# maoqingyu1996/Boosting-Neural-Video-Representation-via-Online-Structural-Reparameteration

Measured on AMD Instinct MI355X. Metric: training frames/sec, Bunny 720p ERB, higher is better.
Workload: dtype f16; 1 GPU; configs[1]: Bunny-shaped 132x3x720x1280 synthetic video, branch_type=ERB, fc_hw_dim 9_16_26, strides 5 2 2 2 2, stem 512_1, lower_width 96, Fusion6, Adam(0.5,0.999), b=1; one independent video per GPU; precision=fp16, hip_graph=False, launch_mode=stream, finite=True

## Files before the change

boosting-neural-video-representation-via-online-structural-reparameteration_amd/csrc/orn_engine.hip:

```cpp
#include "orn_internal.h"
#include <new>
#include <cstdlib>
#include <cassert>

struct LayerBuf {
    float *T, *wf, *bf;
    float *w2t;
    float *dT, *dw1p;
    float *wd32;
    void *mh16;
    float *dw2t;
    float *z, *a;
    float *da;
    uint16_t *xpad;
    uint16_t *zb;
    uint16_t *dypad;
    uint16_t *wb, *wd;
    float *biasp;
    float *wslab;
};

struct orn_engine {
    orn_engine_desc d;
    float *params, *grads, *m, *v;
    const float *gmask;
    const float *tstats;
    float *ws;
    float *pre1, *h1, *pre2, *h2, *dh2;
    float *img, *dimg, *stats;
    float *loss_ws;
    float *dec_ws;
    float *scratch;
    float *head_ws;
    OrnStepCur *cur;
    LayerBuf L[ORN_MAX_LAYERS];
    int Hout, Wout, Cn_last;
    const OrnHalfOps *ops;
    float gs;
    OrnScaleState *sc;
    struct MergeSet {
        int n;
        OrnMergeLayer ml[ORN_MAX_LAYERS];
        int layer[ORN_MAX_LAYERS];
        void *tables;
        int tiles[4];
        void *mh_tables, *mh_host;
    } mset[3];
    int ff;
    float *dxn;
    size_t stem_ws;
    bool stage0;
    hipGraph_t graph, graph_u;
    hipGraphExec_t graph_exec, graph_exec_u;
    const void *g_frames, *g_embeds, *g_sched, *g_cursor, *g_stats;
    int g_slots;
    hipStream_t g_stream;
    hipStream_t side;
    hipEvent_t ev_fork, ev_adam, ev_wgrad, ev_join, ev_below;
    OrnStepCur *cur_side;
    OrnScaleState *sc_side;
    size_t side_lo;
    bool pipe_ok;
    bool side_below;
    bool fork_behind_dgrad;
    int last_smax;
    bool side_busy;
    bool prof;
    hipEvent_t prof_ev[4 * ORN_MAX_LAYERS + 4];
};

#define ORN_GRAPH_UNROLL 4
static_assert(ORN_SCALE_SLOTS >= ORN_GRAPH_UNROLL, "one scale-state entry per step of the unrolled graph");

static inline size_t al(size_t floats) { return orn_align(floats * 4) / 4; }

static hipEvent_t orn_engine::*const SIDE_EVENTS[] = {&orn_engine::ev_fork, &orn_engine::ev_adam, &orn_engine::ev_wgrad, &orn_engine::ev_join,
                                                      &orn_engine::ev_below};

static constexpr int ORN_LAST_SMAX = 24;

static void drop_graphs(orn_engine *e)
{
    if (e->graph_exec) { (void)hipGraphExecDestroy(e->graph_exec); e->graph_exec = nullptr; }
    if (e->graph) { (void)hipGraphDestroy(e->graph); e->graph = nullptr; }
    if (e->graph_exec_u) { (void)hipGraphExecDestroy(e->graph_exec_u); e->graph_exec_u = nullptr; }
    if (e->graph_u) { (void)hipGraphDestroy(e->graph_u); e->graph_u = nullptr; }
}

extern "C" size_t orn_conv3x3_ps_silu_bwd_ws_bytes(int B, int C, int O, int H, int W);
extern "C" size_t orn_erb_merge_bwd_ws_bytes(int C, int O);
extern "C" size_t orn_head_bwd_ws_bytes(int B, int C, int H, int W);
extern "C" size_t orn_loss_ws_bytes(int B, int Ch, int H, int W);

static int check_desc(const orn_engine_desc *d)
{
    ORN_REQUIRE(d, "engine: null desc");
    ORN_REQUIRE(d->n_layers >= 1 && d->n_layers <= ORN_MAX_LAYERS, "engine: n_layers=%d out of range", d->n_layers);
    ORN_REQUIRE(d->precision >= 0 && d->precision <= 2, "engine: precision %d not built", d->precision);
    ORN_REQUIRE(d->embed_len > 0 && d->stem_dim > 0 && d->fc_h > 0 && d->fc_w > 0 && d->fc_dim > 0, "engine: bad stem geometry");
    int C = d->fc_dim, H = d->fc_h, W = d->fc_w;
    for (int i = 0; i < d->n_layers; ++i) {
        const orn_layer_desc &l = d->layer[i];
        ORN_REQUIRE(l.C == C && l.H == H && l.W == W,
                    "engine: layer %d geometry (C=%d,H=%d,W=%d) does not chain (expected %d,%d,%d)", i, l.C, l.H, l.W, C, H, W);
        ORN_REQUIRE(l.s >= 1 && l.O > 0 && l.O % (l.s * l.s) == 0, "engine: layer %d: O=%d not divisible by s^2", i, l.O);
        ORN_REQUIRE(l.w3x3 >= 0 && l.b3x3 >= 0, "engine: layer %d: missing 3x3 weight/bias", i);
        if (d->erb)
            ORN_REQUIRE(l.w3x1 >= 0 && l.b3x1 >= 0 && l.w1x3 >= 0 && l.b1x3 >= 0 && l.w1 >= 0 && l.w2 >= 0 && l.w3 >= 0,
                        "engine: layer %d: missing ERB branch tensors", i);
        C = l.O / (l.s * l.s); H *= l.s; W *= l.s;
    }
    ORN_REQUIRE(d->n_params > 0 && d->n_params % 4 == 0, "engine: n_params must be a positive multiple of 4");
    ORN_REQUIRE(d->loss_type >= 0 && d->loss_type <= 2, "engine: bad loss_type %d", d->loss_type);
    return 0;
}

#define ORN_FAST_C 96
static bool layer_is_fast(const orn_layer_desc &l)
{
    return l.C == ORN_FAST_C && l.O % 96 == 0 && l.O % (l.s * l.s) == 0;
}

static int first_fast_layer(const orn_engine_desc *d)
{
    if (d->precision == 0) return d->n_layers;
    const orn_layer_desc &last = d->layer[d->n_layers - 1];
    const int cn = last.O / (last.s * last.s);
    if (!(cn == 32 || cn == 64 || cn == 96 || cn == 128)) return d->n_layers;
    int ff = d->n_layers;
    while (ff > 0 && layer_is_fast(d->layer[ff - 1])) --ff;
    if (ff > 0 && ff < d->n_layers) {
        const orn_layer_desc &l = d->layer[ff - 1];
        if (l.C < ORN_FAST_C && l.O % 96 == 0 && l.O % (l.s * l.s) == 0) --ff;
    }
    return ff;
}

static size_t layout(const orn_engine_desc *d, orn_engine *e)
{
    size_t off = 0;
    const int ff = first_fast_layer(d);
    float *dxn = nullptr;
    float *base = e ? e->ws : nullptr;
    auto take = [&](size_t floats) { float *p = base ? base + off : nullptr; off += al(floats); return p; };
    const int Nout = d->fc_h * d->fc_w * d->fc_dim;
    float *pre1 = take(d->stem_dim), *h1 = take(d->stem_dim), *pre2 = take(Nout), *h2 = take(Nout), *dh2 = take(Nout);
    size_t scratch = orn_stem_bwd_ws_floats(1, d->stem_dim, Nout);
    LayerBuf L[ORN_MAX_LAYERS] = {};
    int Cn = d->fc_dim, H = d->fc_h, W = d->fc_w;
    for (int i = 0; i < d->n_layers; ++i) {
        const orn_layer_desc &l = d->layer[i];
        const size_t wsz = (size_t)l.O * l.C * 9;
        if (d->erb) {
            L[i].T = take(wsz); L[i].wf = take(wsz); L[i].bf = take(l.O);
            L[i].w2t = (2 * l.C * 9 * 4 * 4 <= 64 * 1024) ? take((size_t)9 * l.O * 2 * l.C) : nullptr;
            L[i].dT = take(wsz); L[i].dw1p = take((size_t)9 * 2 * l.C * l.C);
            if (d->precision != 0) {
                L[i].mh16 = take((orn_merge_h16_layer_halfs(l.C, l.O) + 1) / 2);
                L[i].dw2t = take((size_t)9 * l.O * 2 * l.C);
            }
        }
        Cn = l.O / (l.s * l.s); H = l.H * l.s; W = l.W * l.s;
        const size_t asz = (size_t)Cn * H * W;
        size_t s1;
        if (i < ff) {
            L[i].z = take(asz); L[i].a = take(asz); L[i].da = take(asz);
            L[i].wd32 = take(wsz);
            s1 = orn_conv3x3_ps_silu_bwd_ws_bytes(1, l.C, l.O, l.H, l.W) / 4;
            const size_t s0 = al(orn_stem_bwd_ws_floats(1, d->stem_dim, Nout)) + (size_t)orn_stage0_slabs(l.O, l.s) * l.C * l.H * l.W;
            if (s0 > s1) s1 = s0;
        } else {
            const size_t wpz = (size_t)l.O * ORN_FAST_C * 9 + 96 * ORN_FAST_C;
            L[i].xpad = (uint16_t *)take(((size_t)(l.H + 2) * (l.W + 2) * ORN_FAST_C + 1) / 2);
            L[i].zb = (uint16_t *)take((asz + 1) / 2);
            L[i].dypad = (uint16_t *)take(((size_t)(l.H + 2) * (l.W + 2) * l.O + 128 + 1) / 2);
            L[i].wb = (uint16_t *)take((wpz + 1) / 2);
            L[i].wd = (uint16_t *)take((wpz + 1) / 2);
            L[i].biasp = take(l.O);
            L[i].wslab = take(orn_half_ops_bf16()->wgrad_ws_floats(l.H, l.W, l.O));
            const OrnHalfOps *ops = orn_half_ops_bf16();
            if (i == ff) dxn = take((size_t)l.H * l.W * ORN_FAST_C * ops->dgrad_f32_slabs(l.H, l.W, l.O));
            s1 = al(ops->wgrad_ws_floats(l.H, l.W, l.O));
            const size_t sd = (size_t)l.H * l.W * ORN_FAST_C * ops->dgrad_f32_slabs(l.H, l.W, l.O);
            if (ops->dgrad_f32_slabs(l.H, l.W, l.O) > 1 && sd > s1) s1 = sd;
        }
        if (d->erb) { const size_t s2 = orn_erb_merge_bwd_ws_bytes(l.C, l.O) / 4; if (s2 > s1) s1 = s2; }
        if (s1 > scratch) scratch = s1;
    }
    const size_t isz = (size_t)3 * H * W;
    float *img = take(isz), *dimg = take(isz), *stats = take(8);
    float *loss_ws = take(orn_loss_ws_bytes(1, 3, H, W) / 4);
    const size_t s3 = (ff < d->n_layers) ? orn_half_ops_bf16()->head_bwd_ws_floats(Cn) : orn_head_bwd_ws_bytes(1, Cn, H, W) / 4;
    if (s3 > scratch) scratch = s3;
    float *scr = take(scratch);
    const orn_layer_desc &ll = d->layer[d->n_layers - 1];
    float *head_ws = (ff < d->n_layers) ? take(orn_half_ops_bf16()->head_bwd_ws_floats(Cn))
                   : (ll.s == 2 ? take((size_t)(orn_head_bwd_fused_f32_blocks(ll.H, ll.W) + 1) * (3 * Cn + 3)) : nullptr);
    float *cur = take((sizeof(OrnStepCur) * ORN_GRAPH_UNROLL + 3) / 4 + 16);
    float *scs = take(sizeof(OrnScaleState) * ORN_SCALE_SLOTS / 4);
    float *mtab[3], *mhtab[3];
    for (int k = 0; k < 3; ++k) {
        mtab[k] = d->erb ? take(orn_merge_group_bytes() / 4) : nullptr;
        mhtab[k] = (d->erb && d->precision != 0) ? take(orn_merge_h16_table_bytes() / 4) : nullptr;
    }
    float *cur_side = take((sizeof(OrnStepCur) + 3) / 4 + 16);
    float *sc_side = take(sizeof(OrnScaleState) / 4 + 16);
    float *dec_ws = take(ORN_DECODE_WS_FLOATS);
    if (e) {
        e->pre1 = pre1; e->h1 = h1; e->pre2 = pre2; e->h2 = h2; e->dh2 = dh2;
        e->img = img; e->dimg = dimg; e->stats = stats; e->loss_ws = loss_ws; e->scratch = scr; e->head_ws = head_ws;
        e->cur = (OrnStepCur *)cur;
        e->sc = (OrnScaleState *)scs;
        for (int i = 0; i < d->n_layers; ++i) e->L[i] = L[i];
        e->Hout = H; e->Wout = W; e->Cn_last = Cn;
        e->ff = ff; e->dxn = dxn;
        e->stem_ws = al(orn_stem_bwd_ws_floats(1, d->stem_dim, Nout));
        const orn_layer_desc &l0 = d->layer[0];
        e->stage0 = d->precision != 0 && ff == 1 && d->n_layers > 1 && orn_stage0_supported(l0.C, l0.O, l0.H, l0.W, l0.s);
        for (int k = 0; k < 3; ++k) { e->mset[k].tables = mtab[k]; e->mset[k].mh_tables = mhtab[k]; }
        e->cur_side = (OrnStepCur *)cur_side;
        e->sc_side = (OrnScaleState *)sc_side;
        e->dec_ws = dec_ws;
    }
    return off * 4;
}

extern "C" size_t orn_engine_ws_bytes(const orn_engine_desc *d)
{
    if (check_desc(d) != 0) return 0;
    return layout(d, nullptr);
}

extern "C" int orn_engine_create(const orn_engine_desc *d, float *params, float *grads, float *adam_m, float *adam_v,
                                 void *ws, size_t ws_bytes, orn_engine **out)
{
    ORN_TRY(check_desc(d));
    ORN_REQUIRE(params && out && ws, "engine_create: null pointer");
    ORN_REQUIRE(((uintptr_t)params | (uintptr_t)grads | (uintptr_t)adam_m | (uintptr_t)adam_v | (uintptr_t)ws) % 256 == 0,
                "engine_create: arenas and workspace must be 256-byte aligned");
    const size_t need = layout(d, nullptr);
    if (ws_bytes < need) {
        orn_set_error("engine_create: workspace %zu < %zu", ws_bytes, need);
        return ORN_E_WS;
    }
    ORN_TRY(orn_loss_init());
    orn_engine *e = new (std::nothrow) orn_engine();
    ORN_REQUIRE(e, "engine_create: out of host memory");
    e->d = *d;
    e->params = params; e->grads = grads; e->m = adam_m; e->v = adam_v;
    e->gmask = nullptr;
    e->tstats = nullptr;
    e->ws = (float *)ws;
    e->graph = nullptr; e->graph_exec = nullptr; e->graph_u = nullptr; e->graph_exec_u = nullptr;
    e->prof = false;
    for (int k = 0; k < 3; ++k) { e->mset[k].n = 0; e->mset[k].mh_host = nullptr; }
    e->side = nullptr;
    for (auto ev : SIDE_EVENTS) e->*ev = nullptr;
    e->pipe_ok = false; e->side_busy = false; e->side_lo = 0;
    for (int i = 0; i < 4 * ORN_MAX_LAYERS + 4; ++i) e->prof_ev[i] = nullptr;
    e->ops = (d->precision == 2) ? orn_half_ops_f16() : orn_half_ops_bf16();
    e->gs = (d->precision == 2) ? 1048576.0f : 1.0f;
    layout(d, e);
    {
        hipError_t rc = hipMemset(ws, 0, need);
        if (rc == hipSuccess) rc = hipDeviceSynchronize();
        if (rc != hipSuccess) { orn_set_error("engine_create: hipMemset failed: %s", hipGetErrorString(rc)); delete e; return (int)rc; }
        OrnScaleState s0[ORN_SCALE_SLOTS] = {};
        for (int r = 0; r < ORN_SCALE_SLOTS; ++r) { s0[r].gs = e->gs; s0[r].inv_gs = 1.0f / e->gs; s0[r].gs_max = e->gs; }
        rc = hipMemcpy(e->sc, s0, sizeof(s0), hipMemcpyHostToDevice);
        if (rc == hipSuccess) rc = hipMemcpy(e->sc_side, s0, sizeof(OrnScaleState), hipMemcpyHostToDevice);
        if (rc != hipSuccess) { orn_set_error("engine_create: scale state upload failed: %s", hipGetErrorString(rc)); delete e; return (int)rc; }
    }
    {
        const int nl = d->n_layers;
        const orn_layer_desc &ll = d->layer[nl - 1];
        bool ok = d->precision != 0 && e->ff < nl - 1 && grads && adam_m && adam_v;
        if (ok) {
            const int64_t lo_all[9] = {ll.w3x3, ll.b3x3, ll.w3x1, ll.b3x1, ll.w1x3, ll.b1x3, ll.w1, ll.w2, ll.w3};
            int64_t lo = d->n_params;
            for (int k = 0; k < (d->erb ? 9 : 2); ++k) if (lo_all[k] >= 0 && lo_all[k] < lo) lo = lo_all[k];
            ok = d->head_w >= lo && d->head_b >= lo && d->stem_w0 < lo && d->stem_b0 < lo && d->stem_w1 < lo && d->stem_b1 < lo && lo % 64 == 0;
            for (int i = 0; i < nl - 1 && ok; ++i) {
                const orn_layer_desc &l = d->layer[i];
                const int64_t o[9] = {l.w3x3, l.b3x3, l.w3x1, l.b3x1, l.w1x3, l.b1x3, l.w1, l.w2, l.w3};
                for (int k = 0; k < (d->erb ? 9 : 2); ++k) ok = ok && o[k] < lo;
            }
            e->side_lo = (size_t)lo;
        }
        if (ok) {
            hipError_t rc = hipStreamCreateWithFlags(&e->side, hipStreamNonBlocking);
            for (auto ev : SIDE_EVENTS)
                if (rc == hipSuccess) rc = hipEventCreateWithFlags(&(e->*ev), hipEventDisableTiming | hipEventDisableSystemFence);
            if (rc != hipSuccess) { orn_set_error("engine_create: side stream: %s", hipGetErrorString(rc)); orn_engine_destroy(e); return (int)rc; }
        }
        e->pipe_ok = ok;
        e->last_smax = ok ? ORN_LAST_SMAX : 0;
        e->side_below = ok && nl - 2 > e->ff;
        e->fork_behind_dgrad = e->side_below;
    }
    if (!d->erb)
        for (int i = 0; i < d->n_layers; ++i) {
            e->L[i].T = nullptr;
            e->L[i].wf = params + d->layer[i].w3x3;
            e->L[i].bf = params + d->layer[i].b3x3;
        }
    else {
        auto fill = [&](int i, OrnMergeLayer &m, bool half_in_S) {
            const orn_layer_desc &l = d->layer[i];
            m.C = l.C; m.O = l.O;
            m.w3x3 = params + l.w3x3; m.w3x1 = params + l.w3x1; m.w1x3 = params + l.w1x3;
            m.w1 = params + l.w1; m.w2 = params + l.w2; m.w3 = params + l.w3;
            m.T = e->L[i].T; m.wf = e->L[i].wf; m.w2t = e->L[i].w2t;
            m.b3x3 = params + l.b3x3; m.b1x3 = params + l.b1x3; m.b3x1 = params + l.b3x1; m.bf = e->L[i].bf;
            m.g = grads ? grads + l.w3x3 : nullptr;
            m.dT = e->L[i].dT; m.dw1p = e->L[i].dw1p;
            m.dw2 = grads ? grads + l.w2 : nullptr; m.dw3 = grads ? grads + l.w3 : nullptr;
            m.dw2t = e->L[i].dw2t;
            m.half_kind = 0; m.s2 = l.s * l.s; m.Cp = ORN_FAST_C; m.wb = m.wd = nullptr; m.biasp = nullptr;
            if (i >= e->ff && half_in_S) {
                m.half_kind = d->precision; m.wb = e->L[i].wb; m.wd = e->L[i].wd; m.biasp = e->L[i].biasp;
            }
        };
        const int nl = d->n_layers;
        for (int k = 0; k < (e->pipe_ok ? 3 : 1); ++k) {
            orn_engine::MergeSet &ms = e->mset[k];
            const int i0 = k == 2 ? nl - 1 : 0, i1 = k == 1 ? nl - 1 : nl;
            ms.n = 0;
            void *bufs[ORN_MAX_LAYERS];
            for (int i = i0; i < i1; ++i) {
                fill(i, ms.ml[ms.n], k == 2 || !e->stage0);
                bufs[ms.n] = e->L[i].mh16;
                ms.layer[ms.n++] = i;
            }
            int rc = orn_merge_groups_build(ms.tables, ms.n, ms.ml, d->precision != 0);
            if (rc == 0 && d->precision != 0) {
                ms.mh_host = malloc(orn_merge_h16_host_bytes());
                rc = ms.mh_host ? orn_merge_h16_build(ms.mh_tables, ms.mh_host, ms.n, ms.ml, bufs, k == 2 ? e->sc_side : e->sc) : ORN_E_ARG;
            }
            if (rc != 0) { orn_engine_destroy(e); return rc; }
            for (int q = 0; q < 4; ++q) ms.tiles[q] = orn_merge_group_tiles(q, ms.n, ms.ml);
        }
    }
    *out = e;
    return 0;
}

extern "C" void orn_engine_destroy(orn_engine *e)
{
    if (!e) return;
    drop_graphs(e);
    for (int i = 0; i < 4 * ORN_MAX_LAYERS + 4; ++i)
        if (e->prof_ev[i]) (void)hipEventDestroy(e->prof_ev[i]);
    if (e->side) { (void)hipStreamSynchronize(e->side); (void)hipStreamDestroy(e->side); }
    for (auto ev : SIDE_EVENTS) if (e->*ev) (void)hipEventDestroy(e->*ev);
    for (int k = 0; k < 3; ++k) free(e->mset[k].mh_host);
    delete e;
}

extern "C" int orn_engine_set_grad_mask(orn_engine *e, const float *mask)
{
    ORN_REQUIRE(e, "engine_set_grad_mask: null engine");
    ORN_REQUIRE((uintptr_t)mask % 16 == 0, "engine_set_grad_mask: mask must be 16-byte aligned");
    e->gmask = mask;
    drop_graphs(e);
    return 0;
}

extern "C" int orn_engine_set_target_stats(orn_engine *e, const float *stats)
{
    ORN_REQUIRE(e, "engine_set_target_stats: null engine");
    ORN_REQUIRE((uintptr_t)stats % 16 == 0, "engine_set_target_stats: stats must be 16-byte aligned");
    e->tstats = stats;
    drop_graphs(e);
    return 0;
}

extern "C" int orn_engine_scale_state(orn_engine *e, float *out8)
{
    ORN_REQUIRE(e && out8, "engine_scale_state: null pointer");
    OrnScaleState sa[ORN_SCALE_SLOTS];
    hipError_t rc = hipDeviceSynchronize();
    if (rc == hipSuccess) rc = hipMemcpy(sa, e->sc, sizeof(sa), hipMemcpyDeviceToHost);
    if (rc != hipSuccess) { orn_set_error("engine_scale_state: %s", hipGetErrorString(rc)); return (int)rc; }
    const OrnScaleState &s = sa[0];
    int any = 0;
    for (int r = 0; r < ORN_SCALE_SLOTS; ++r) any |= sa[r].flag;
    any |= s.late_skipped != s.late_seen ? 1 : 0;
    out8[0] = s.gs; out8[1] = s.inv_gs; out8[2] = s.gs_max; out8[3] = (float)any; out8[4] = (float)s.skipped;
    out8[5] = (float)s.good; out8[6] = (float)s.backoffs; out8[7] = (float)s.late_skipped;
    return 0;
}

extern "C" int orn_engine_set_grad_scale(orn_engine *e, float gs, float gs_max)
{
    ORN_REQUIRE(e && gs >= 1.0f, "engine_set_grad_scale: scale must be >= 1");
    OrnScaleState sa[ORN_SCALE_SLOTS];
    hipError_t rc = hipDeviceSynchronize();
    if (rc == hipSuccess) rc = hipMemcpy(sa, e->sc, sizeof(sa), hipMemcpyDeviceToHost);
    for (int r = 0; r < ORN_SCALE_SLOTS; ++r) {
        sa[r].gs = gs; sa[r].inv_gs = 1.0f / gs;
        if (gs_max > 0.f) sa[r].gs_max = gs_max;
    }
    sa[0].good = 0;
    if (rc == hipSuccess) rc = hipMemcpy(e->sc, sa, sizeof(sa), hipMemcpyHostToDevice);
    if (rc != hipSuccess) { orn_set_error("engine_set_grad_scale: %s", hipGetErrorString(rc)); return (int)rc; }
    return 0;
}

extern "C" int orn_engine_fused_kernel(orn_engine *e, int layer, const float **wf, const float **bf)
{
    ORN_REQUIRE(e && wf && bf && layer >= 0 && layer < e->d.n_layers, "engine_fused_kernel: bad arguments");
    *wf = e->L[layer].wf;
    *bf = e->L[layer].bf;
    return 0;
}

__global__ void k_advance(const orn_step_sched *__restrict__ sched, int32_t *cursor, int32_t n_slots, double beta1,
                          double beta2, OrnStepCur *cur_all, int count, OrnScaleState *sc)
{
    const int32_t c0 = *cursor;
    __shared__ int32_t skipped;
    if (threadIdx.x == 0) {
        int nflag = 0;
        for (int r = 0; r < ORN_SCALE_SLOTS; ++r)
            if (sc[r].flag) { nflag += 1; sc[r].flag = 0; }
        const int32_t late = __atomic_load_n(&sc->late_skipped, __ATOMIC_RELAXED);
        if (late != sc->late_seen) { nflag += 1; sc->late_seen = late; }
        float gs = sc->gs;
        if (nflag) {
            gs = fmaxf(gs * 0.5f, 1.0f);
            sc->good = 0; sc->backoffs += 1;
        } else {
            sc->good += sc->launched;
            if (sc->good >= ORN_SCALE_GROWTH_INTERVAL && gs < sc->gs_max) { gs *= 2.0f; sc->good = 0; }
        }
        sc->launched = count;
        for (int r = 0; r < ORN_SCALE_SLOTS; ++r) { sc[r].gs = gs; sc[r].inv_gs = 1.0f / gs; }
        skipped = sc->skipped;
    }
    __syncthreads();
    if (blockIdx.x == 0 && (int)threadIdx.x < count) {
        const int32_t c = c0 + threadIdx.x;
        OrnStepCur *cur = cur_all + threadIdx.x;
        orn_step_sched s = sched[c];
        s.step = max(s.step - skipped, 1);
        cur->frame = s.frame;
        cur->step = s.step;
        cur->lr = s.lr;
        const double bc1 = 1.0 - pow(beta1, (double)s.step), bc2 = 1.0 - pow(beta2, (double)s.step);
        cur->step_size = (float)((double)s.lr / bc1);
        cur->sqrt_bc2 = (float)sqrt(bc2);
        cur->slot = n_slots > 0 ? c % n_slots : 0;
        if (threadIdx.x == 0) *cursor = c0 + count;
    }
}

static bool f32_head_on_z(const orn_engine *e)
{
    const orn_engine_desc &d = e->d;
    return e->ff >= d.n_layers && e->head_ws && d.layer[d.n_layers - 1].s == 2;
}

static int slab_cap(const orn_engine *e, int i) { return i == e->d.n_layers - 1 ? e->last_smax : 0; }

static OrnPrepLayer prep_layer(const orn_engine *e, int i)
{
    const orn_layer_desc &l = e->d.layer[i];
    return OrnPrepLayer{e->L[i].wf, e->L[i].bf, l.O, l.C, l.s, e->L[i].wb, e->L[i].wd, e->L[i].biasp, ORN_FAST_C};
}

static OrnWgradJob wgrad_job(const orn_engine *e, int i)
{
    const orn_layer_desc &l = e->d.layer[i];
    return OrnWgradJob{e->L[i].xpad, e->L[i].dypad, l.H, l.W, l.C, l.O, l.s, e->L[i].wslab, slab_cap(e, i)};
}

static OrnWgradReduce wgrad_reduce(const orn_engine *e, int i, OrnScaleState *sc)
{
    const orn_layer_desc &l = e->d.layer[i];
    return OrnWgradReduce{e->L[i].wslab, l.H, l.W, l.C, l.O, l.s, 1.0f / e->gs, e->grads + l.w3x3, e->grads + l.b3x3, sc, slab_cap(e, i)};
}

enum { MERGE_NONE = -1 };
static int forward(orn_engine *e, const float *embeds, const int *row_idx, bool keep_z, hipStream_t st, int set = 0, bool head = true)
{
    const bool merge = set != MERGE_NONE;
    const orn_engine_desc &d = e->d;
    const int Nout = d.fc_h * d.fc_w * d.fc_dim;
    float *P = e->params;
    const OrnLinearJob lin1 = {embeds, row_idx, (size_t)d.embed_len, P + d.stem_w0, P + d.stem_b0, 1, d.embed_len, d.stem_dim, e->pre1, e->h1};
    const OrnLinearJob lin2 = {e->h1, nullptr, 0, P + d.stem_w1, P + d.stem_b1, 1, d.stem_dim, Nout, e->pre2, e->h2};
    const float *x = e->h2;
    const int nl = d.n_layers, ff = e->ff;
    const void *pack_t = nullptr;
    int pack_t_blocks = 0;
    if (d.erb && merge) {
        const orn_engine::MergeSet &ms = e->mset[set];
        int pk_par = 0, pk_t = 0;
        const void *pk = (keep_z && ms.mh_host) ? orn_merge_h16_pack(ms.mh_host, &pk_par, &pk_t) : nullptr;
        ORN_TRY(orn_launch_w2_transpose(ms.n, ms.ml, st, pk, pk_par));
        ORN_TRY(orn_launch_merge_group_linear(ms.tables, 0, ms.tiles[0], lin1, st));
        ORN_TRY(orn_launch_merge_group_linear(ms.tables, 1, ms.tiles[1], lin2, st, e->stage0 ? nullptr : pk, e->stage0 ? 0 : pk_t));
        pack_t = e->stage0 ? pk : nullptr; pack_t_blocks = e->stage0 ? pk_t : 0;
    } else {
        ORN_TRY(orn_launch_linear_silu(lin1.x, lin1.row_idx, lin1.row_stride, lin1.w, lin1.bias, 1, lin1.K, lin1.N, lin1.pre, lin1.y, st));
        ORN_TRY(orn_launch_linear_silu(lin2.x, nullptr, 0, lin2.w, lin2.bias, 1, lin2.K, lin2.N, lin2.pre, lin2.y, st));
    }
    if (ff < nl && !d.erb && merge) {
        OrnPrepLayer pl[ORN_MAX_LAYERS];
        const int np = (set == 1 ? nl - 1 : nl) - ff;
        for (int i = ff; i < ff + np; ++i) pl[i - ff] = prep_layer(e, i);
        ORN_TRY(e->ops->prep_all(np, pl, st));
    }
    OrnHeadFuse hf = {};
    for (int i = 0; i < nl; ++i) {
        const orn_layer_desc &l = d.layer[i];
        LayerBuf &b = e->L[i];
        if (i < ff) {
            if (e->prof) (void)hipEventRecord(e->prof_ev[2 * i], st);
            if (e->stage0) {
                OrnPrepLayer pl[ORN_MAX_LAYERS];
                int np = 0;
                if (d.erb && merge)
                    for (int j = ff; j < (set == 1 ? nl - 1 : nl); ++j) pl[np++] = prep_layer(e, j);
                ORN_TRY(orn_launch_stage0_fwd(x, b.wf, b.bf, l.C, l.O, l.H, l.W, l.s, keep_z ? b.z : nullptr, e->L[1].xpad, ORN_FAST_C,
                                              d.precision, st, np, pl, pack_t, pack_t_blocks));
            }
            else
            {
                const bool z_only = keep_z && i == nl - 1 && f32_head_on_z(e);
                ORN_TRY(orn_launch_conv3x3_f32(x, b.wf, b.bf, 1, l.C, l.O, l.H, l.W, l.s, 1, keep_z ? b.z : nullptr, z_only ? nullptr : b.a, st, nullptr));
            }
            if (e->prof) (void)hipEventRecord(e->prof_ev[2 * i + 1], st);
            x = b.a;
        } else {
            if (i == ff && !e->stage0) ORN_TRY(e->ops->to_nhwc(x, l.C, ORN_FAST_C, l.H, l.W, b.xpad, st));
            if (e->prof) (void)hipEventRecord(e->prof_ev[2 * i], st);
            const bool last = (i + 1 == nl);
            if (e->side_busy && i + 3 == nl && e->side_below) ORN_HIP(hipStreamWaitEvent(st, e->ev_below, 0));
            if (e->side_busy && i + 2 == nl) ORN_HIP(hipStreamWaitEvent(st, e->ev_wgrad, 0));
            if (e->side_busy && last) { ORN_HIP(hipStreamWaitEvent(st, e->ev_join, 0)); e->side_busy = false; }
            if (last) hf = OrnHeadFuse{P + d.head_w, P + d.head_b, e->img, d.sigmoid, 0};
            ORN_TRY(e->ops->conv_fwd(b.xpad, b.wb, b.biasp, l.H, l.W, ORN_FAST_C, l.O, l.s, b.zb, last ? nullptr : e->L[i + 1].xpad, st, l.C,
                                     last && head ? &hf : nullptr));
            if (e->prof) (void)hipEventRecord(e->prof_ev[2 * i + 1], st);
        }
    }
    if (ff < nl) {
        if (!hf.fused && head)
            ORN_TRY(e->ops->head_fwd(e->L[nl - 1].zb, P + d.head_w, P + d.head_b, e->Cn_last, (size_t)e->Hout * e->Wout, d.sigmoid, e->img, st));
    } else
    {
        const bool z_only = keep_z && f32_head_on_z(e);
        ORN_TRY(orn_launch_head_fwd(z_only ? e->L[nl - 1].z : x, P + d.head_w, P + d.head_b, 1, e->Cn_last, (size_t)e->Hout * e->Wout, d.sigmoid, e->img,
                                    st, z_only));
    }
    return 0;
}

extern "C" int orn_engine_decode(orn_engine *e, const float *embed, float *img, void *stream)
{
    ORN_REQUIRE(e && embed && img, "engine_decode: null pointer");
    hipStream_t st = (hipStream_t)stream;
    ORN_TRY(forward(e, embed, nullptr, false, st));
    hipError_t rc = hipMemcpyAsync(img, e->img, (size_t)3 * e->Hout * e->Wout * 4, hipMemcpyDeviceToDevice, st);
    if (rc != hipSuccess) { orn_set_error("engine_decode: copy failed: %s", hipGetErrorString(rc)); return (int)rc; }
    return 0;
}

extern "C" int orn_engine_decode_frames(orn_engine *e, const float *embeds, const int32_t *rows, int32_t n, const float *targets,
                                        uint8_t *rgb8, float *img, float *stats, void *stream)
{
    ORN_REQUIRE(e && embeds, "engine_decode_frames: null engine / embeds");
    ORN_REQUIRE(n >= 0 && (rows || n == 0), "engine_decode_frames: n=%d frames need a device array of n row indices", n);
    ORN_REQUIRE(rgb8 || img || stats, "engine_decode_frames: no output asked for (rgb8, img and stats are all null)");
    ORN_REQUIRE(!stats || targets, "engine_decode_frames: stats need targets");
    assert(!e->side_busy);
    hipStream_t st = (hipStream_t)stream;
    const orn_engine_desc &d = e->d;
    const size_t HW = (size_t)e->Hout * e->Wout;
    const bool fast = e->ff < d.n_layers;
    if (stats && n > 0) ORN_HIP(hipMemsetAsync(e->dec_ws + 2 * ORN_DECODE_MAX_BLOCKS, 0, 64 * 4, st));
    for (int32_t k = 0; k < n; ++k) {
        ORN_TRY(forward(e, embeds, rows + k, false, st, k == 0 ? 0 : MERGE_NONE, false));
        const OrnDecodeOut o = {targets, rows + k, rgb8 ? rgb8 + (size_t)k * HW * 3 : nullptr, img ? img + (size_t)k * HW * 3 : nullptr,
                                stats ? stats + (size_t)k * 4 : nullptr, e->dec_ws};
        if (fast)
            ORN_TRY(e->ops->decode_out(e->L[d.n_layers - 1].zb, e->params + d.head_w, e->params + d.head_b, e->Cn_last, HW, d.sigmoid, o, st));
        else
            ORN_TRY(orn_launch_decode_out_f32(e->img, HW, o, st));
    }
    return 0;
}

static OrnMergeMisc merge_misc(const orn_engine *e, int i)
{
    const orn_layer_desc &l = e->d.layer[i];
    float *G = e->grads;
    OrnMergeMisc m = {};
    m.C = l.C; m.O = l.O;
    m.g = G + l.w3x3; m.dbf = G + l.b3x3; m.dw1p = e->L[i].dw1p;
    m.d3x1 = G + l.w3x1; m.db3x1 = G + l.b3x1; m.d1x3 = G + l.w1x3; m.db1x3 = G + l.b1x3;
    m.dw1 = G + l.w1;
    if (e->d.precision != 0) { m.dw2t = e->L[i].dw2t; m.dw2 = G + l.w2; }
    return m;
}

static int side_branch_backward(orn_engine *e, hipStream_t st)
{
    const orn_engine_desc &d = e->d;
    const int nl = d.n_layers;
    float *G = e->grads;
    hipStream_t sd = e->side;
    OrnScaleState *sc = e->sc_side;
    ORN_HIP(hipEventRecord(e->ev_fork, st));
    ORN_HIP(hipStreamWaitEvent(sd, e->ev_fork, 0));
    if (e->side_below) {
        const OrnWgradJob wb = wgrad_job(e, nl - 2);
        ORN_TRY(e->ops->wgrad_batch(1, &wb, sd, nullptr, nullptr, 1));
        ORN_HIP(hipEventRecord(e->ev_below, sd));
    }
    const OrnWgradJob wj = wgrad_job(e, nl - 1);
    const OrnHeadFinish hf = {e->head_ws, e->ops->head_bwd_blocks(e->Hout, e->Wout), e->Cn_last, 1.0f / e->gs, G + d.head_w, G + d.head_b, sc};
    ORN_TRY(e->ops->wgrad_batch(1, &wj, sd, &hf, nullptr, 1));
    ORN_HIP(hipEventRecord(e->ev_wgrad, sd));
    const OrnWgradReduce wr = wgrad_reduce(e, nl - 1, sc);
    ORN_TRY(e->ops->wgrad_reduce_all(1, &wr, sd, nullptr));
    if (d.erb) {
        const orn_engine::MergeSet &ms = e->mset[2];
        ORN_TRY(orn_launch_merge_h16_bwd(ms.mh_tables, ms.mh_host, sd, sc));
        const OrnMergeMisc mm = merge_misc(e, nl - 1);
        ORN_TRY(orn_launch_merge_bwd_tail_all(1, &mm, sd));
    }
    return 0;
}

static int side_branch_update(orn_engine *e, bool more)
{
    const orn_engine_desc &d = e->d;
    const int nl = d.n_layers;
    hipStream_t sd = e->side;
    const size_t lo = e->side_lo;
    ORN_HIP(hipStreamWaitEvent(sd, e->ev_adam, 0));
    ORN_TRY(orn_launch_adam(e->params + lo, e->grads + lo, e->m + lo, e->v + lo, (size_t)d.n_params - lo, 0.0, 1, e->cur_side, d.beta1, d.beta2,
                            d.eps, 1.0f, sd, e->gmask ? e->gmask + lo : nullptr, e->sc_side, nullptr, nullptr, false, e->sc));
    const void *packs = nullptr;
    if (more && d.erb) {
        const orn_engine::MergeSet &ms = e->mset[2];
        const OrnLinearJob none = {};
        ORN_TRY(orn_launch_w2_transpose(ms.n, ms.ml, sd));
        ORN_TRY(orn_launch_merge_group_linear(ms.tables, 0, ms.tiles[0], none, sd));
        ORN_TRY(orn_launch_merge_group_linear(ms.tables, 1, ms.tiles[1], none, sd));
        packs = ms.mh_host;
    } else if (more) {
        const OrnPrepLayer pl = prep_layer(e, nl - 1);
        ORN_TRY(e->ops->prep_all(1, &pl, sd));
    }
    ORN_HIP(hipEventRecord(e->ev_join, sd));
    if (packs) {
        ORN_TRY(orn_launch_merge_h16_pack_jobs(packs, 1, sd));
        ORN_TRY(orn_launch_merge_h16_pack_jobs(packs, 2, sd));
    }
    e->side_busy = true;
    return 0;
}

static int fast_weight_grads(orn_engine *e, hipStream_t st, bool pipe, OrnScaleState *sc, const OrnStemL2Job *l2job, const OrnStemW0Job *w0job)
{
    const orn_engine_desc &d = e->d;
    const int nl = d.n_layers, ff = e->ff;
    OrnWgradJob wj[ORN_MAX_LAYERS];
    int nj = 0;
    const int n_main = pipe ? nl - 1 : nl;
    for (int i = n_main - 1; i >= ff; --i) {
        if (pipe && i == nl - 2 && e->side_below) continue;
        wj[nj++] = wgrad_job(e, i);
    }
    const OrnHeadFinish hf = {e->head_ws, e->ops->head_bwd_blocks(e->Hout, e->Wout), e->Cn_last, 1.0f / e->gs, e->grads + d.head_w, e->grads + d.head_b, sc};
    if (e->prof) (void)hipEventRecord(e->prof_ev[4 * ORN_MAX_LAYERS], st);
    ORN_TRY(e->ops->wgrad_batch(nj, wj, st, pipe ? nullptr : &hf, l2job, 0));
    if (e->prof) (void)hipEventRecord(e->prof_ev[4 * ORN_MAX_LAYERS + 1], st);
    OrnWgradReduce wr[ORN_MAX_LAYERS];
    for (int i = ff; i < n_main; ++i) wr[i - ff] = wgrad_reduce(e, i, sc);
    if (e->prof) (void)hipEventRecord(e->prof_ev[4 * ORN_MAX_LAYERS + 2], st);
    if (pipe && e->side_below) ORN_HIP(hipStreamWaitEvent(st, e->ev_below, 0));
    ORN_TRY(e->ops->wgrad_reduce_all(n_main - ff, wr, st, w0job));
    if (e->prof) (void)hipEventRecord(e->prof_ev[4 * ORN_MAX_LAYERS + 3], st);
    return 0;
}

static int merge_backward(orn_engine *e, const orn_engine::MergeSet &ms, hipStream_t st, OrnScaleState *sc)
{
    if (e->d.precision != 0) {
        ORN_TRY(orn_launch_merge_h16_bwd(ms.mh_tables, ms.mh_host, st, sc));
    } else {
        ORN_TRY(orn_launch_merge_group(ms.tables, 2, ms.tiles[2], st));
        ORN_TRY(orn_launch_merge_group(ms.tables, 3, ms.tiles[3], st));
    }
    OrnMergeMisc mm[ORN_MAX_LAYERS];
    for (int k = 0; k < ms.n; ++k) mm[k] = merge_misc(e, ms.layer[k]);
    ORN_TRY(orn_launch_merge_bwd_tail_all(ms.n, mm, st));
    return 0;
}

struct StepOpts {
    int advance = 1;
    int cur = 0;
    bool pipe = false;
    bool more = false;
};

static int train_step(orn_engine *e, const float *frames, const float *embeds, const orn_step_sched *sched,
                      int32_t *cursor, float *stats_out, int32_t n_slots, hipStream_t st, const StepOpts &o = StepOpts())
{
    const orn_engine_desc &d = e->d;
    const bool pipe = o.pipe;
    float *P = e->params, *G = e->grads;
    const int Nout = d.fc_h * d.fc_w * d.fc_dim;
    const size_t HWo = (size_t)e->Hout * e->Wout;
    OrnStepCur *cur = e->cur + o.cur;
    if (o.advance > 0) {
        hipLaunchKernelGGL(k_advance, dim3(1), dim3(64), 0, st, sched, cursor, n_slots, d.beta1, d.beta2, e->cur, o.advance, e->sc );
        ORN_LAUNCH_CHECK("advance");
    }
    OrnScaleState *const sc = e->sc + o.cur;
    const int *fidx = &cur->frame;
    ORN_TRY(forward(e, embeds, fidx, true, st, (pipe && e->side_busy) ? 1 : 0));
    const int nl = d.n_layers, ff = e->ff;
    OrnLossFinalJob fin = {};
    ORN_TRY(orn_launch_loss(e->img, frames, fidx, 3 * HWo, 1, 3, e->Hout, e->Wout, d.loss_type, 1.0f, e->stats, e->dimg,
                            e->loss_ws, st, cur, stats_out, sc, d.loss_type == ORN_LOSS_FUSION6 ? e->tstats : nullptr,
                            ff < nl ? &fin : nullptr));
    if (pipe) { fin.cur_copy = e->cur_side; fin.sc_copy = e->sc_side; }
    if (ff < nl)
        ORN_TRY(e->ops->head_bwd(e->L[nl - 1].zb, P + d.head_w, e->img, e->dimg, e->Cn_last, e->Hout, e->Wout, d.sigmoid,
                                 d.layer[nl - 1].s, e->gs, e->L[nl - 1].dypad, nullptr, nullptr, e->head_ws, st, sc, &fin));
    const bool head_fused32 = f32_head_on_z(e);
    const OrnHeadBwdFuse hfuse = {P + d.head_w, e->img, e->dimg, d.sigmoid, G + d.head_w, G + d.head_b, e->head_ws};
    if (ff >= nl && !head_fused32)
        ORN_TRY(orn_launch_head_bwd(e->L[nl - 1].a, P + d.head_w, e->img, e->dimg, 1, e->Cn_last, HWo, d.sigmoid, e->L[nl - 1].da,
                                    G + d.head_w, G + d.head_b, e->scratch, st));
    if (ff >= nl) {
        const float *wfs[ORN_MAX_LAYERS]; float *wds[ORN_MAX_LAYERS]; int Os[ORN_MAX_LAYERS], Cs[ORN_MAX_LAYERS];
        for (int i = 0; i < nl; ++i) { wfs[i] = e->L[i].wf; wds[i] = e->L[i].wd32; Os[i] = d.layer[i].O; Cs[i] = d.layer[i].C; }
        ORN_TRY(orn_launch_flip_transpose_all(nl, wfs, wds, Os, Cs, st));
    }
    for (int i = nl - 1; i >= 0; --i) {
        const orn_layer_desc &l = d.layer[i];
        LayerBuf &b = e->L[i];
        const float *x = (i == 0) ? e->h2 : e->L[i - 1].a;
        float *dx = (i == 0) ? e->dh2 : e->L[i - 1].da;
        if (e->prof) (void)hipEventRecord(e->prof_ev[2 * ORN_MAX_LAYERS + 2 * i], st);
        if (i >= ff) {
            if (i > ff) {
                float *part = e->ops->dgrad_f32_slabs(l.H, l.W, l.O) > 1 ? e->scratch : nullptr;
                ORN_TRY(e->ops->conv_dgrad(b.dypad, b.wd, l.H, l.W, l.O, l.C, e->L[i - 1].zb, e->L[i - 1].dypad, d.layer[i - 1].s,
                                           part, st, l.C));
            } else {
                ORN_TRY(e->ops->conv_dgrad(b.dypad, b.wd, l.H, l.W, l.O, ORN_FAST_C, nullptr, nullptr, 1, e->dxn, st, l.C));
                if (!e->stage0)
                ORN_TRY(e->ops->to_nchw_f32(e->dxn, l.C, ORN_FAST_C, l.H, l.W, e->ops->dgrad_f32_slabs(l.H, l.W, l.O), 1.0f / e->gs, dx,
                                            st, sc));
            }
        } else if (e->stage0) {
            const orn_layer_desc &l1 = d.layer[1];
            ORN_TRY(orn_launch_stage0_bwd(x, b.wf, b.z, e->dxn, e->ops->dgrad_f32_slabs(l1.H, l1.W, l1.O), ORN_FAST_C, 1.0f / e->gs, l.C, l.O,
                                          l.H, l.W, l.s, e->scratch + e->stem_ws, nullptr, G + l.w3x3, G + l.b3x3, st, sc));
        } else
        ORN_TRY(orn_launch_conv_bwd_f32(x, b.wf, b.z, b.da, 1, l.C, l.O, l.H, l.W, l.s, dx, G + l.w3x3, G + l.b3x3, e->scratch, st,
                                        (i == nl - 1 && head_fused32) ? &hfuse : nullptr, ff >= nl ? b.wd32 : nullptr));
        if (e->prof) (void)hipEventRecord(e->prof_ev[2 * ORN_MAX_LAYERS + 2 * i + 1], st);
        if (pipe && e->fork_behind_dgrad && i == nl - 1) ORN_TRY(side_branch_backward(e, st));
    }
    OrnStemW0Job w0job;
    OrnStemL2Job l2job;
    const bool defer_w0 = ff < nl;
    ORN_TRY(orn_launch_stem_bwd(embeds, fidx, d.embed_len, P + d.stem_w1, e->pre1, e->h1, e->pre2,
                                e->stage0 ? e->scratch + e->stem_ws : e->dh2, 1, d.embed_len, d.stem_dim, Nout, G + d.stem_w0,
                                G + d.stem_b0, G + d.stem_w1, G + d.stem_b1, e->scratch, st,
                                e->stage0 ? orn_stage0_slabs(d.layer[0].O, d.layer[0].s) : 1, defer_w0 ? &w0job : nullptr, defer_w0 ? &l2job : nullptr));
    if (ff < nl) ORN_TRY(fast_weight_grads(e, st, pipe, sc, &l2job, &w0job));
    if (pipe && !e->fork_behind_dgrad) ORN_TRY(side_branch_backward(e, st));
    if (d.erb) ORN_TRY(merge_backward(e, e->mset[pipe ? 1 : 0], st, sc));
    if (pipe) {
        ORN_TRY(orn_launch_adam(P, G, e->m, e->v, e->side_lo, 0.0, 1, cur, d.beta1, d.beta2, d.eps, 1.0f, st, e->gmask, sc, e->sc, e->sc_side));
        ORN_HIP(hipEventRecord(e->ev_adam, st));
        return side_branch_update(e, o.more);
    }
    ORN_TRY(orn_launch_adam(P, G, e->m, e->v, (size_t)d.n_params, 0.0, 1, cur, d.beta1, d.beta2, d.eps, 1.0f, st, e->gmask, sc, e->sc));
    return 0;
}

extern "C" int orn_engine_train_step(orn_engine *e, const float *frames, const float *embeds,
                                     const orn_step_sched *sched, int32_t *cursor, float *stats_out, int32_t n_slots,
                                     void *stream)
{
    ORN_REQUIRE(e && frames && embeds && sched && cursor, "engine_train_step: null pointer");
    ORN_REQUIRE(e->grads && e->m && e->v, "engine_train_step: engine was created without grads / Adam arenas");
    return train_step(e, frames, embeds, sched, cursor, stats_out, n_slots, (hipStream_t)stream);
}

extern "C" int orn_engine_train_steps(orn_engine *e, const float *frames, const float *embeds, const orn_step_sched *sched,
                                      int32_t *cursor, float *stats_out, int32_t n_slots, int32_t n_steps, void *stream)
{
    ORN_REQUIRE(e && frames && embeds && sched && cursor && n_steps >= 0, "engine_train_steps: bad arguments");
    ORN_REQUIRE(e->grads && e->m && e->v, "engine_train_steps: engine was created without grads / Adam arenas");
    hipStream_t st = (hipStream_t)stream;
    int rc = 0;
    StepOpts o;
    o.pipe = e->pipe_ok;
    for (int k = 0; k < n_steps && rc == 0; ++k) {
        o.more = k + 1 < n_steps;
        rc = train_step(e, frames, embeds, sched, cursor, stats_out, n_slots, st, o);
    }
    if (e->side_busy) {
        const hipError_t hrc = hipStreamWaitEvent(st, e->ev_join, 0);
        e->side_busy = false;
        if (hrc != hipSuccess && rc == 0) { orn_set_error("engine_train_steps: join: %s", hipGetErrorString(hrc)); rc = (int)hrc; }
    }
    return rc;
}

extern "C" int orn_engine_profile_step(orn_engine *e, const float *frames, const float *embeds, const orn_step_sched *sched,
                                       int32_t *cursor, float *stats_out, int32_t n_slots, float *ms_out, void *stream)
{
    ORN_REQUIRE(e && frames && embeds && sched && cursor && ms_out, "engine_profile_step: null pointer");
    ORN_REQUIRE(e->grads && e->m && e->v, "engine_profile_step: engine was created without grads / Adam arenas");
    hipStream_t st = (hipStream_t)stream;
    const int nl = e->d.n_layers;
    for (int i = 0; i < 4 * ORN_MAX_LAYERS + 4; ++i)
        if (!e->prof_ev[i]) {
            hipError_t rc = hipEventCreate(&e->prof_ev[i]);
            if (rc != hipSuccess) { orn_set_error("engine_profile_step: hipEventCreate: %s", hipGetErrorString(rc)); return (int)rc; }
        }
    e->prof = true;
    const int trc = train_step(e, frames, embeds, sched, cursor, stats_out, n_slots, st);
    e->prof = false;
    if (trc != 0) return trc;
    hipError_t rc = hipStreamSynchronize(st);
    if (rc != hipSuccess) { orn_set_error("engine_profile_step: sync: %s", hipGetErrorString(rc)); return (int)rc; }
    auto span = [&](int a, float *out) -> int {
        float ms = 0.f;
        hipError_t r = hipEventElapsedTime(&ms, e->prof_ev[a], e->prof_ev[a + 1]);
        if (r != hipSuccess) { orn_set_error("engine_profile_step: elapsed: %s", hipGetErrorString(r)); return (int)r; }
        *out = ms;
        return 0;
    };
    const bool fast = e->ff < nl;
    for (int i = 0; i < nl; ++i) {
        ORN_TRY(span(2 * i, &ms_out[i]));
        ORN_TRY(span(2 * ORN_MAX_LAYERS + 2 * i, &ms_out[nl + i]));
    }
    ms_out[2 * nl] = ms_out[2 * nl + 1] = 0.f;
    if (fast) {
        ORN_TRY(span(4 * ORN_MAX_LAYERS, &ms_out[2 * nl]));
        ORN_TRY(span(4 * ORN_MAX_LAYERS + 2, &ms_out[2 * nl + 1]));
    }
    return 0;
}

extern "C" int orn_engine_train_steps_graph(orn_engine *e, const float *frames, const float *embeds,
                                            const orn_step_sched *sched, int32_t *cursor, float *stats_out,
                                            int32_t n_slots, int32_t n_steps, void *stream)
{
    ORN_REQUIRE(e && frames && embeds && sched && cursor && n_steps >= 0, "engine_train_steps_graph: bad arguments");
    ORN_REQUIRE(e->grads && e->m && e->v, "engine_train_steps_graph: engine was created without grads / Adam arenas");
    hipStream_t st = (hipStream_t)stream;
    const bool same = e->graph_exec && e->g_frames == frames && e->g_embeds == embeds && e->g_sched == sched &&
                      e->g_cursor == cursor && e->g_stats == stats_out && e->g_slots == n_slots && e->g_stream == st;
    if (!same) {
        drop_graphs(e);
        for (int pass = 0; pass < 2; ++pass) {
            const int reps = pass == 0 ? 1 : ORN_GRAPH_UNROLL;
            hipGraph_t *g = pass == 0 ? &e->graph : &e->graph_u;
            hipGraphExec_t *ge = pass == 0 ? &e->graph_exec : &e->graph_exec_u;
            hipError_t rc = hipStreamBeginCapture(st, hipStreamCaptureModeThreadLocal);
            if (rc != hipSuccess) { orn_set_error("graph: BeginCapture failed: %s", hipGetErrorString(rc)); return (int)rc; }
            int trc = 0;
            for (int r = 0; r < reps && trc == 0; ++r) {
                StepOpts o;
                o.advance = r == 0 ? reps : 0;
                o.cur = r;
                trc = train_step(e, frames, embeds, sched, cursor, stats_out, n_slots, st, o);
            }
            rc = hipStreamEndCapture(st, g);
            if (trc != 0) { if (*g) { (void)hipGraphDestroy(*g); *g = nullptr; } return trc; }
            if (rc != hipSuccess) { orn_set_error("graph: EndCapture failed: %s", hipGetErrorString(rc)); return (int)rc; }
            rc = hipGraphInstantiate(ge, *g, nullptr, nullptr, 0);
            if (rc != hipSuccess) { orn_set_error("graph: Instantiate failed: %s", hipGetErrorString(rc)); return (int)rc; }
        }
        e->g_frames = frames; e->g_embeds = embeds; e->g_sched = sched; e->g_cursor = cursor; e->g_stats = stats_out;
        e->g_slots = n_slots; e->g_stream = st;
    }
    int left = n_steps;
    if (left > ORN_GRAPH_UNROLL) {
        hipError_t rc = hipGraphLaunch(e->graph_exec, st);
        if (rc != hipSuccess) { orn_set_error("graph: Launch failed: %s", hipGetErrorString(rc)); return (int)rc; }
        left -= 1;
    }
    while (left > 0) {
        const bool big = left >= ORN_GRAPH_UNROLL;
        hipError_t rc = hipGraphLaunch(big ? e->graph_exec_u : e->graph_exec, st);
        if (rc != hipSuccess) { orn_set_error("graph: Launch failed: %s", hipGetErrorString(rc)); return (int)rc; }
        left -= big ? ORN_GRAPH_UNROLL : 1;
    }
    return 0;
}
```

boosting-neural-video-representation-via-online-structural-reparameteration_amd/csrc/orn_internal.h:

```cpp
#pragma once
#include "orn_common.h"

int orn_launch_linear_silu(const float *x, const int *row_idx, size_t row_stride, const float *w, const float *b,
                           int B, int K, int N, float *pre, float *y, hipStream_t st);
int orn_launch_stem_bwd(const float *embed, const int *row_idx, size_t row_stride, const float *w1, const float *pre1,
                        const float *h1, const float *pre2, const float *dh2, int B, int E, int Hd, int Nout,
                        float *dw0, float *db0, float *dw1, float *db1, float *ws, hipStream_t st, int dh2_nslab = 1,
                        OrnStemW0Job *defer_w0 = nullptr,
                        OrnStemL2Job *defer_l2 = nullptr);
size_t orn_stem_bwd_ws_floats(int B, int Hd, int Nout);
int orn_launch_head_fwd(const float *a, const float *w, const float *b, int B, int C, size_t HW, int sigmoid,
                        float *out, hipStream_t st, bool z_input = false);
int orn_launch_head_bwd(const float *a, const float *w, const float *out, const float *dout, int B, int C, size_t HW,
                        int sigmoid, float *da, float *dw, float *db, float *ws, hipStream_t st);
int orn_launch_adam(float *p, const float *g, float *m, float *v, size_t n, double lr, int step, const OrnStepCur *sp,
                    double beta1, double beta2, double eps, float inv_gscale, hipStream_t st, const float *gmask = nullptr,
                    OrnScaleState *sc = nullptr,
                    OrnScaleState *sc_master = nullptr,
                    OrnScaleState *mirror = nullptr,
                    bool count_skip = true,
                    OrnScaleState *late = nullptr);

bool orn_stage0_supported(int C, int O, int H, int W, int s);
int orn_stage0_slabs(int O, int s);
struct OrnPrepLayer;
int orn_launch_stage0_fwd(const float *x, const float *wf, const float *bf, int C, int O, int H, int W, int s, float *z,
                          void *xpad_next, int Cp, int precision, hipStream_t st, int n_prep = 0, const OrnPrepLayer *prep = nullptr,
                          const void *pack = nullptr, int pack_t_blocks = 0);
int orn_launch_stage0_bwd(const float *x, const float *wf, const float *z, const float *dxn, int nslab, int Cp, float inv_gs, int C,
                          int O, int H, int W, int s, float *slabs, float *dx, float *dwf, float *dbf, hipStream_t st,
                          const OrnScaleState *sc = nullptr);

int orn_launch_merge_fwd(const float *w3x3, const float *b3x3, const float *w3x1, const float *b3x1,
                         const float *w1x3, const float *b1x3, const float *w1, const float *w2, const float *w3,
                         int C, int O, float *T, float *wf, float *bf, hipStream_t st);
int orn_launch_merge_bwd(const float *g, const float *dbf, const float *w1, const float *w2, const float *w3,
                         const float *T, int C, int O, float *d3x3, float *db3x3, float *d3x1, float *db3x1,
                         float *d1x3, float *db1x3, float *dw1, float *dw2, float *dw3, float *ws, hipStream_t st);

struct OrnMergeLayer {
    int C, O;
    const float *w3x3, *w3x1, *w1x3, *w1, *w2, *w3;
    const float *b3x3, *b1x3, *b3x1; float *bf;
    float *T, *wf;
    float *w2t;
    const float *g;
    float *dT, *dw1p, *dw2, *dw3;
    float *dw2t;
    int half_kind, s2, Cp;
    void *wb, *wd;
    float *biasp;
};
size_t orn_merge_group_bytes();
int orn_launch_w2_transpose(int n_layers, const OrnMergeLayer *L, hipStream_t st, const void *pack = nullptr, int par_blocks = 0);
int orn_merge_groups_build(void *dev_tables, int n_layers, const OrnMergeLayer *L, int bwd_h16);
int orn_merge_group_tiles(int which, int n_layers, const OrnMergeLayer *L);
int orn_launch_merge_group(const void *dev_tables, int which, int tiles, hipStream_t st);
int orn_launch_merge_group_linear(const void *dev_tables, int which, int tiles, const OrnLinearJob &job, hipStream_t st,
                                  const void *pack = nullptr, int pack_blocks = 0);
int orn_launch_merge_bias(const float *b3x3, const float *b1x3, const float *b3x1, int O, float *bf, hipStream_t st);
int orn_launch_merge_bwd_tail(const float *g, const float *dbf, int C, int O, float *d3x3, float *db3x3, float *d3x1,
                              float *db3x1, float *d1x3, float *db1x3, const float *dw1p, float *dw1, hipStream_t st);

size_t orn_merge_h16_layer_halfs(int C, int O);
size_t orn_merge_h16_table_bytes();
size_t orn_merge_h16_host_bytes();
int orn_merge_h16_build(void *dev_tables, void *host, int n_layers, const OrnMergeLayer *L, void *const *bufs, OrnScaleState *sc);
int orn_launch_merge_h16_bwd(const void *dev_tables, const void *host, hipStream_t st, OrnScaleState *sc = nullptr);
const void *orn_merge_h16_pack(const void *host, int *par_blocks, int *t_blocks);
int orn_launch_merge_h16_pack_jobs(const void *host, int which, hipStream_t st);

struct OrnMergeMisc {
    int C, O;
    const float *b3x3, *b1x3, *b3x1; float *bf;
    const float *g, *dbf, *dw1p;
    float *d3x1, *db3x1, *d1x3, *db1x3, *dw1;
    const float *dw2t; float *dw2;
};
int orn_launch_merge_bias_all(int n, const OrnMergeMisc *L, hipStream_t st);
int orn_launch_merge_bwd_tail_all(int n, const OrnMergeMisc *L, hipStream_t st);

int orn_launch_conv3x3_f32(const float *x, const float *w, const float *bias, int B, int C, int O, int H, int W,
                           int s, int epi, float *z, float *out, hipStream_t st, float *split_ws);
struct OrnHeadBwdFuse { const float *w, *out, *dout; int sigmoid; float *dw, *db, *hws; };
int orn_launch_conv_bwd_f32(const float *x, const float *wf, const float *z, const float *da, int B, int C, int O,
                            int H, int W, int s, float *dx, float *dwf, float *dbf, float *ws, hipStream_t st,
                            const OrnHeadBwdFuse *head = nullptr, const float *wd_ready = nullptr);
int orn_launch_flip_transpose_all(int n, const float *const *wf, float *const *wd, const int *O, const int *C, hipStream_t st);
int orn_head_bwd_fused_f32_blocks(int H, int W);
int orn_launch_head_bwd_fused_f32(const float *z, const float *w, const float *out, const float *dout, int Cn, int H, int W,
                                  int sigmoid, float *dy, float *dbp, float *dw, float *db, float *hws, hipStream_t st);

int orn_loss_init();
int orn_launch_loss(const float *pred, const float *target, const int *frame_idx, size_t frame_stride, int B, int Ch,
                    int H, int W, int loss_type, float loss_scale, float *stats, float *dpred, float *ws,
                    hipStream_t st, const OrnStepCur *cur = nullptr, float *ring = nullptr, OrnScaleState *sc = nullptr,
                    const float *tstats = nullptr,
                    OrnLossFinalJob *defer = nullptr);

struct OrnPrepLayer { const float *wf, *bf; int O, C, s; void *wb, *wd; float *biasp; int Cp; };
struct OrnWgradReduce { const float *slabs; int H, W, C, O, s; float gscale; float *dwf, *dbf; OrnScaleState *sc; int smax; };
struct OrnHeadFinish { const float *partial; int blocks, C; float gscale; float *dw, *db; OrnScaleState *sc; };
struct OrnWgradJob { const void *xpad, *dypad; int H, W, C, O, s; float *slabs; int smax; };
struct OrnHeadFuse { const float *w, *b; float *out; int sigmoid; int fused; };
#define ORN_DECODE_MAX_BLOCKS 8192
#define ORN_DECODE_WS_FLOATS (2 * ORN_DECODE_MAX_BLOCKS + 64)
struct OrnDecodeOut { const float *targets; const int32_t *row; uint8_t *rgb8; float *img, *stats; float *ws; };
int orn_launch_decode_out_f32(const float *src, size_t HW, const OrnDecodeOut &o, hipStream_t st);
struct OrnHalfOps {
    int (*conv_fwd)(const void *xpad, const void *wb, const float *bias_p, int H, int W, int Cin, int O, int s, void *z, void *apad,
                    hipStream_t st, int c_real, OrnHeadFuse *head);
    int (*conv_dgrad)(const void *dypad, const void *wd, int H, int W, int O, int C, const void *zprev, void *dyprev, int sp,
                      float *dx_f32, hipStream_t st, int c_real);
    size_t (*wgrad_ws_floats)(int H, int W, int O);
    int (*wgrad)(const void *xpad, const void *dypad, int H, int W, int C, int O, int s, float gscale, float *slabs, float *dwf,
                 float *dbf, hipStream_t st);
    int (*wgrad_batch)(int n, const OrnWgradJob *J, hipStream_t st, const OrnHeadFinish *hf, const OrnStemL2Job *l2, int side);
    int (*wgrad_reduce_all)(int n, const OrnWgradReduce *L, hipStream_t st, const OrnStemW0Job *w0);
    int (*prep_all)(int n, const OrnPrepLayer *L, hipStream_t st);
    int (*to_nhwc)(const float *src, int C, int Cp, int H, int W, void *dst, hipStream_t st);
    int (*to_nchw_f32)(const float *src, int C, int Cp, int H, int W, int nslab, float scale, float *dst, hipStream_t st, const OrnScaleState *sc);
    int (*dgrad_f32_slabs)(int H, int W, int O);
    int (*head_fwd)(const void *z, const float *w, const float *b, int C, size_t HW, int sigmoid, float *out, hipStream_t st);
    size_t (*head_bwd_ws_floats)(int C);
    int (*head_bwd_blocks)(int H, int W);
    int (*head_bwd)(const void *z, const float *w, const float *out, const float *dout, int C, int H, int W, int sigmoid, int sp,
                    float gs_up, void *dypad, float *dw, float *db, float *ws, hipStream_t st, const OrnScaleState *sc,
                    const OrnLossFinalJob *fin);
    int (*decode_out)(const void *z, const float *w, const float *b, int C, size_t HW, int sigmoid, const OrnDecodeOut &o, hipStream_t st);
};
const OrnHalfOps *orn_half_ops_bf16();
const OrnHalfOps *orn_half_ops_f16();
```

boosting-neural-video-representation-via-online-structural-reparameteration_amd/csrc/orn_merge.hip:

```cpp
#include "orn_internal.h"
#include "orn_merge_pack.h"
#include <cstdlib>
#include <type_traits>

struct GemmP {
    const float *A, *B;
    float *C;
    int M, N, K;
    long sam, sak;
    long sbk, sbn;
    long scm, scn;
    long ba, bb, bc;
    int a_kfast, b_nfast;
    int a_vec, b_vec;
    int epi;
    const float *w3x3, *w1x3, *w3x1;
    int Cch;
    const float *b3x3, *b1x3, *b3x1;
    float *bf;
    float sa, sb, so;
    void *wb, *wd;
    float *biasp;
    int half_kind, s2, Cn, Cp;
};

typedef __attribute__((ext_vector_type(16))) float f32x16;

#define GT 64
#define GK 64
#define GLDA (GK + 1)
#define GLDB (GT + 4)

__device__ __forceinline__ void gemm_body(const GemmP &p, int bx, int by, int bz)
{
    __shared__ float As[GT][GLDA];
    __shared__ float Bs[GK][GLDB];
    const int t = threadIdx.x, lane = t & 63, wave = t >> 6;
    const int l31 = lane & 31, hh = lane >> 5;
    const int wm = wave >> 1, wn = wave & 1;
    const int m0 = by * GT, n0 = bx * GT;
    const float *A = p.A + (long)bz * p.ba;
    const float *B = p.B + (long)bz * p.bb;
    float *C = p.C + (long)bz * p.bc;
    f32x16 acc;
#pragma unroll
    for (int r = 0; r < 16; ++r) acc[r] = 0.f;

    constexpr int NE = GT * GK / 256;
    float ra[NE], rb[NE];
    const int tf = t & 63, tv = t >> 6;
    const int M = p.M, N = p.N, K = p.K;
    const int sam = (int)p.sam, sak = (int)p.sak, sbk = (int)p.sbk, sbn = (int)p.sbn;
    const bool akf = p.a_kfast, bnf = p.b_nfast;
    auto gload1 = [&](int k0, int i) {
        {
            const int v = tv + 4 * i;
            const int am = akf ? v : tf, ak = k0 + (akf ? tf : v);
            const int bn = bnf ? tf : v, bk = k0 + (bnf ? v : tf);
            const float va = A[__mul24(min(m0 + am, M - 1), sam) + __mul24(min(ak, K - 1), sak)];
            const float vb = B[__mul24(min(bk, K - 1), sbk) + __mul24(min(n0 + bn, N - 1), sbn)];
            ra[i] = va;
            rb[i] = vb;
        }
    };
    auto gload = [&](int k0) {
#pragma unroll
        for (int i = 0; i < NE; ++i) gload1(k0, i);
    };
    gload(0);
    for (int k0 = 0; k0 < p.K; k0 += GK) {
        __syncthreads();
#pragma unroll
        for (int i = 0; i < NE; ++i) {
            const int v = tv + 4 * i;
            As[akf ? v : tf][akf ? tf : v] = (k0 + (akf ? tf : v) < K) ? ra[i] : 0.f;
            Bs[bnf ? v : tf][bnf ? tf : v] = (k0 + (bnf ? v : tf) < K) ? rb[i] : 0.f;
        }
        __syncthreads();
        if (k0 + GK < p.K) gload(k0 + GK);
        const float *ap = &As[wm * 32 + l31][hh];
        const float *bp = &Bs[hh][wn * 32 + l31];
#pragma unroll
        for (int kk = 0; kk < GK; kk += 2)
            acc = __builtin_amdgcn_mfma_f32_32x32x2f32(ap[kk], bp[kk * GLDB], acc, 0, 0, 0);
    }
    const int gn = n0 + wn * 32 + l31;
    if (p.epi == 1 && p.bf && bx == 0 && wn == 0 && l31 == 0) {
#pragma unroll
        for (int reg = 0; reg < 16; ++reg) {
            const int gm = m0 + wm * 32 + (reg & 3) + 8 * (reg >> 2) + 4 * hh;
            if (gm < p.M) {
                const float b = p.b3x3[gm] + (p.b1x3[gm] + p.b3x1[gm]);
                p.bf[gm] = b;
                if (p.half_kind) p.biasp[(gm % p.s2) * p.Cn + gm / p.s2] = b;
            }
        }
    }
    if (gn >= p.N) return;
#pragma unroll
    for (int reg = 0; reg < 16; ++reg) {
        const int gm = m0 + wm * 32 + (reg & 3) + 8 * (reg >> 2) + 4 * hh;
        if (gm >= p.M) continue;
        float r = acc[reg];
        if (p.epi == 1) {
            const int c = gn / 9, ij = gn % 9, ii = ij / 3, jj = ij % 3;
            const long oc = (long)gm * p.Cch + c;
            const float p13 = (ii == 1) ? p.w1x3[oc * 3 + jj] : 0.f;
            const float p31 = (jj == 1) ? p.w3x1[oc * 3 + ii] : 0.f;
            r = (p.w3x3[(long)gm * p.N + gn] + (p13 + p31)) + r;
            if (p.half_kind) {
                const int op = (gm % p.s2) * p.Cn + gm / p.s2;
                const size_t ib = ((size_t)ij * p.M + op) * p.Cp + c, id = ((size_t)(8 - ij) * p.Cp + c) * p.M + op;
                if (p.half_kind == 1) {
                    const __bf16 h = (__bf16)r;
                    reinterpret_cast<__bf16 *>(p.wb)[ib] = h;
                    reinterpret_cast<__bf16 *>(p.wd)[id] = h;
                } else {
                    const _Float16 h = (_Float16)r;
                    reinterpret_cast<_Float16 *>(p.wb)[ib] = h;
                    reinterpret_cast<_Float16 *>(p.wd)[id] = h;
                }
            }
        }
        C[(long)gm * p.scm + (long)gn * p.scn] = r;
    }
}


#define G2_KC 32
#ifndef G2_ABL
#define G2_ABL 0
#endif
template <int WM, int WN>
struct G2Regs { float4 a[WM], b[WN]; };

#ifdef ORN_MERGE_STAMP
__device__ unsigned long long g_mst[128];
extern "C" __attribute__((visibility("default"))) int orn_debug_merge_stamps(unsigned long long *out128)
{
    return (int)hipMemcpyFromSymbol(out128, HIP_SYMBOL(g_mst), sizeof(g_mst));
}
#define MST_NOW(t_) do { __builtin_amdgcn_sched_barrier(0); asm volatile("s_memtime %0\n\ts_waitcnt lgkmcnt(0)" : "=s"(t_) :: "memory"); __builtin_amdgcn_sched_barrier(0); } while (0)
#else
#define MST_NOW(t_) do { } while (0)
#endif

template <int I, int N, class F>
__device__ __forceinline__ void g2_sfor(F &&f)
{
    if constexpr (I < N) {
        f(std::integral_constant<int, I>{});
        g2_sfor<I + 1, N>(f);
    }
}

template <int WM, int WN, bool AVEC, bool BVEC>
__device__ __forceinline__ void gemm_body2v(const GemmP &p, int bx, int by, int bz, float *lds)
{
    constexpr int BM = 32 * WM, BN = 32 * WN;
    constexpr int STAGE = BM * G2_KC + G2_KC * BN;
    constexpr int BCH = BN / 4;
    const int t = threadIdx.x, lane = t & 63, wave = t >> 6;
    const int l31 = lane & 31, hh = lane >> 5;
    const int wm = wave / WN, wn = wave - wm * WN;
    const int m0 = by * BM, n0 = bx * BN;
    const float *A = p.A + (long)bz * p.ba;
    const float *B = p.B + (long)bz * p.bb;
    float *C = p.C + (long)bz * p.bc;
    const int M = p.M, N = p.N, K = p.K;
    const int sam = (int)p.sam, sak = (int)p.sak, sbk = (int)p.sbk;
    constexpr bool avec = AVEC;
    static_assert(BVEC, "B is always loaded 16 bytes at a time");
    f32x16 acc;
#pragma unroll
    for (int r = 0; r < 16; ++r) acc[r] = 0.f;
    const unsigned a_bytes = ((unsigned)(M - 1) * (unsigned)sam + (unsigned)(K - 1) * (unsigned)sak + 1u) * 4u;
    const unsigned b_bytes = ((unsigned)(K - 1) * (unsigned)sbk + (unsigned)N) * 4u;
    const auto rA = __builtin_amdgcn_make_buffer_rsrc(const_cast<float *>(A), 0, a_bytes, 0x00020000);
    const auto rB = __builtin_amdgcn_make_buffer_rsrc(const_cast<float *>(B), 0, b_bytes, 0x00020000);
    int a_dst[WM], b_dst[WN];
    unsigned a_vo[WM][avec ? 1 : 4], b_vo[WN];
#pragma unroll
    for (int i = 0; i < WM; ++i) {
        const int u = t + 256 * i, row = u >> 3, ch = u & 7;
#pragma unroll
        for (int j = 0; j < (avec ? 1 : 4); ++j) a_vo[i][j] = ((unsigned)(m0 + row) * (unsigned)sam + (unsigned)(4 * ch + j) * (unsigned)sak) * 4u;
        a_dst[i] = row * 16 + 4 * ((ch >> 1) ^ ((row >> 2) & 3)) + 2 * (ch & 1);
    }
#pragma unroll
    for (int i = 0; i < WN; ++i) {
        const int u = t + 256 * i, kr = u / BCH, ch = u - kr * BCH;
        b_vo[i] = ((unsigned)kr * (unsigned)sbk + (unsigned)(n0 + 4 * ch)) * 4u;
        b_dst[i] = BM * G2_KC + kr * BN + 4 * ch;
    }
    typedef G2Regs<WM, WN> Regs;
#define G2_LOAD16(rsrc_, vo_, so_) __builtin_bit_cast(float4, __builtin_amdgcn_raw_buffer_load_b128(rsrc_, vo_, so_, 0))
    auto gload_a = [&](Regs &R, int i, int k0) {
        const unsigned so = (unsigned)k0 * (unsigned)sak * 4u;
        if constexpr (avec) {
            R.a[i] = G2_LOAD16(rA, a_vo[i][0], so);
        } else {
            R.a[i].x = __builtin_bit_cast(float, __builtin_amdgcn_raw_buffer_load_b32(rA, a_vo[i][0], so, 0));
            R.a[i].y = __builtin_bit_cast(float, __builtin_amdgcn_raw_buffer_load_b32(rA, a_vo[i][1], so, 0));
            R.a[i].z = __builtin_bit_cast(float, __builtin_amdgcn_raw_buffer_load_b32(rA, a_vo[i][2], so, 0));
            R.a[i].w = __builtin_bit_cast(float, __builtin_amdgcn_raw_buffer_load_b32(rA, a_vo[i][3], so, 0));
        }
    };
    auto gload_b = [&](Regs &R, int i, int k0) {
        R.b[i] = G2_LOAD16(rB, b_vo[i], (unsigned)k0 * (unsigned)sbk * 4u);
    };
    auto lstore_a = [&](const Regs &R, int i, int, float *st) {
        const float4 v = R.a[i];
        float *d = st + a_dst[i];
        *reinterpret_cast<float2 *>(d) = make_float2(v.x, v.z);
        *reinterpret_cast<float2 *>(d + BM * 16) = make_float2(v.y, v.w);
    };
    auto lstore_b = [&](const Regs &R, int i, int, float *st) { *reinterpret_cast<float4 *>(st + b_dst[i]) = R.b[i]; };
    auto gload = [&](Regs &R, int k0) {
#pragma unroll
        for (int i = 0; i < WM; ++i) gload_a(R, i, k0);
#pragma unroll
        for (int i = 0; i < WN; ++i) gload_b(R, i, k0);
    };
    auto lstore = [&](const Regs &R, int k0, float *st) {
#pragma unroll
        for (int i = 0; i < WM; ++i) lstore_a(R, i, k0, st);
#pragma unroll
        for (int i = 0; i < WN; ++i) lstore_b(R, i, k0, st);
    };
    struct Frag { float4 a4[G2_KC / 8]; float b[G2_KC / 2]; };
    const int arow = wm * 32 + l31;
    const int a_rd = hh * (BM * 16) + arow * 16, a_sw = (arow >> 2) & 3;
    const int b_rd = BM * G2_KC + hh * BN + wn * 32 + l31;
    auto fread_piece = [&](Frag &F, const float *st, int pc) {
        if (pc < 2) {
#pragma unroll
            for (int j = 0; j < 2; ++j) F.a4[2 * pc + j] = *reinterpret_cast<const float4 *>(st + a_rd + 4 * ((2 * pc + j) ^ a_sw));
        } else {
#pragma unroll
            for (int j = 0; j < 4; ++j) F.b[4 * (pc - 2) + j] = st[b_rd + (2 * (4 * (pc - 2) + j)) * BN];
        }
    };
    auto fread = [&](Frag &F, const float *st) {
#pragma unroll
        for (int pc = 0; pc < 6; ++pc) fread_piece(F, st, pc);
    };
    const int nreal = (K + G2_KC - 1) / G2_KC, nch = (nreal + 2) / 3 * 3;
    Frag F0, F1, F2;
    Regs R0, R1, R2;
    const int gn = n0 + wn * 32 + l31, gnc = min(gn, N - 1);
    const int ec = gnc / 9, eij = gnc - ec * 9, eii = eij / 3, ejj = eij - eii * 3;
    float base[16];
    if (p.epi == 1) {
#pragma unroll
        for (int reg = 0; reg < 16; ++reg) {
            const int gm = min(m0 + wm * 32 + (reg & 3) + 8 * (reg >> 2) + 4 * hh, p.M - 1);
            const long oc = (long)gm * p.Cch + ec;
            const float p13 = (eii == 1) ? p.w1x3[oc * 3 + ejj] : 0.f;
            const float p31 = (ejj == 1) ? p.w3x1[oc * 3 + eii] : 0.f;
            base[reg] = p.w3x3[(long)gm * p.N + gnc] + (p13 + p31);
        }
    }
    unsigned long long t0 = 0, t1 = 0, t2 = 0, ta = 0, tb = 0, s6 = 0;
    (void)t0; (void)t1; (void)t2; (void)ta; (void)tb; (void)s6;
    MST_NOW(t0);
    gload(R0, 0);
    gload(R1, G2_KC);
    gload(R2, 2 * G2_KC);
    __syncthreads();
    lstore(R0, 0, lds);
    lstore(R1, G2_KC, lds + STAGE);
    gload(R0, 3 * G2_KC);
    __syncthreads();
    fread(F0, lds);
    MST_NOW(t1);
    constexpr int NPC = WM + WN;
    static_assert(2 * NPC + 6 <= G2_KC / 2, "more staging pieces than MFMA slots");
    auto step = [&](Frag &Fcur, Frag &Fnext, Regs &Rold, Regs &Rnew, const float *sr, float *sw, int i) {
        MST_NOW(ta);
        const int k_st = (i + 2) * G2_KC, k_ld = (i + 4) * G2_KC;
        g2_sfor<0, G2_KC / 2>([&](auto sc) {
            constexpr int sl = decltype(sc)::value;
            acc = __builtin_amdgcn_mfma_f32_32x32x2f32(Fcur.a4[sl >> 2][sl & 3], Fcur.b[sl], acc, 0, 0, 0);
            if constexpr (sl < NPC && !(G2_ABL & 1)) {
                if constexpr (sl < WM) gload_a(Rnew, sl, k_ld); else gload_b(Rnew, sl - WM, k_ld);
            } else if constexpr (sl >= NPC && sl < NPC + 6 && !(G2_ABL & 4)) {
                fread_piece(Fnext, sr, sl - NPC);
            } else if constexpr (sl >= NPC + 6 && sl < 2 * NPC + 6 && !(G2_ABL & 2)) {
                constexpr int j = sl - NPC - 6;
                if constexpr (j < WM) lstore_a(Rold, j, k_st, sw); else lstore_b(Rold, j - WM, k_st, sw);
            }
            __builtin_amdgcn_sched_barrier(0);
        });
        if constexpr (!(G2_ABL & 8)) __syncthreads();
        MST_NOW(tb);
#ifdef ORN_MERGE_STAMP
        s6 += tb - ta;
#endif
    };
    float *S0 = lds, *S1 = lds + STAGE, *S2 = lds + 2 * STAGE;
    for (int i = 0; i < nch; i += 3) {
        step(F0, F1, R2, R1, S1, S2, i);
        step(F1, F2, R0, R2, S2, S0, i + 1);
        step(F2, F0, R1, R0, S0, S1, i + 2);
    }
    MST_NOW(t2);
    if (p.epi == 1 && p.bf && bx == 0 && wn == 0 && l31 == 0) {
#pragma unroll
        for (int reg = 0; reg < 16; ++reg) {
            const int gm = m0 + wm * 32 + (reg & 3) + 8 * (reg >> 2) + 4 * hh;
            if (gm < p.M) {
                const float b = p.b3x3[gm] + (p.b1x3[gm] + p.b3x1[gm]);
                p.bf[gm] = b;
                if (p.half_kind) p.biasp[(gm % p.s2) * p.Cn + gm / p.s2] = b;
            }
        }
    }
    if (gn < p.N) {
    if (p.epi == 1) {
        const int c = ec, ij = eij;
#pragma unroll
        for (int reg = 0; reg < 16; ++reg) {
            const int gm = m0 + wm * 32 + (reg & 3) + 8 * (reg >> 2) + 4 * hh;
            if (gm >= p.M) continue;
            const float r = base[reg] + acc[reg];
            if (p.half_kind) {
                const int op = (gm % p.s2) * p.Cn + gm / p.s2;
                const size_t ib = ((size_t)ij * p.M + op) * p.Cp + c, id = ((size_t)(8 - ij) * p.Cp + c) * p.M + op;
                if (p.half_kind == 1) {
                    const __bf16 h = (__bf16)r;
                    reinterpret_cast<__bf16 *>(p.wb)[ib] = h;
                    reinterpret_cast<__bf16 *>(p.wd)[id] = h;
                } else {
                    const _Float16 h = (_Float16)r;
                    reinterpret_cast<_Float16 *>(p.wb)[ib] = h;
                    reinterpret_cast<_Float16 *>(p.wd)[id] = h;
                }
            }
            C[(long)gm * p.scm + (long)gn * p.scn] = r;
        }
    } else {
#pragma unroll
        for (int reg = 0; reg < 16; ++reg) {
            const int gm = m0 + wm * 32 + (reg & 3) + 8 * (reg >> 2) + 4 * hh;
            if (gm < p.M) C[(long)gm * p.scm + (long)gn * p.scn] = acc[reg];
        }
    }
    }
#ifdef ORN_MERGE_STAMP
    {
        unsigned long long t3;
        asm volatile("s_waitcnt vmcnt(0)" ::: "memory");
        MST_NOW(t3);
        if (bx == 0 && by == 0 && bz == 0 && t == 0) {
            unsigned long long *rec = g_mst + 16 * ((K / 32) & 7);
            rec[0] = t3 - t0; rec[1] = t1 - t0; rec[2] = t2 - t1; rec[3] = t3 - t2; rec[4] = s6; rec[5] = nch; rec[6] = M; rec[7] = N; rec[8] = K;
        }
    }
#endif
}
#define G2_LDS_FLOATS (3 * (128 * G2_KC + G2_KC * 32))
#define G2_LDS_BYTES(shape_) ((shape_) == 1 ? 3 * (128 * G2_KC + G2_KC * 32) * 4 : 3 * (64 * G2_KC + G2_KC * 64) * 4)
#define G2_LIN_ROUNDS 4
template <int WM, int WN>
__device__ __forceinline__ void gemm_body2(const GemmP &p, int bx, int by, int bz, float *lds)
{
    if (p.a_vec) gemm_body2v<WM, WN, true, true>(p, bx, by, bz, lds);
    else gemm_body2v<WM, WN, false, true>(p, bx, by, bz, lds);
}

typedef __attribute__((ext_vector_type(8))) _Float16 f16x8;
#define HK 64
#define HROW (HK * 2 + 16)

__device__ __forceinline__ void gemm_body_h16(const GemmP &p, int bx, int by, int bz)
{
    __shared__ __attribute__((aligned(16))) unsigned char Ah[GT * HROW];
    __shared__ __attribute__((aligned(16))) unsigned char Bh[GT * HROW];
    const int t = threadIdx.x, lane = t & 63, wave = t >> 6;
    const int l31 = lane & 31, hh = lane >> 5;
    const int wm = wave >> 1, wn = wave & 1;
    const int m0 = by * GT, n0 = bx * GT;
    const float *A = p.A + (long)bz * p.ba;
    const float *B = p.B + (long)bz * p.bb;
    float *C = p.C + (long)bz * p.bc;
    f32x16 acc;
#pragma unroll
    for (int r = 0; r < 16; ++r) acc[r] = 0.f;
    constexpr int NE = GT * HK / 256;
    float ra[NE], rb[NE];
    const int tf = t & 63, tv = t >> 6;
    const int M = p.M, N = p.N, K = p.K;
    const int sam = (int)p.sam, sak = (int)p.sak, sbk = (int)p.sbk, sbn = (int)p.sbn;
    const bool akf = p.a_kfast, bnf = p.b_nfast;
    auto gload = [&](int k0) {
#pragma unroll
        for (int i = 0; i < NE; ++i) {
            const int v = tv + 4 * i;
            const int am = akf ? v : tf, ak = k0 + (akf ? tf : v);
            const int bn = bnf ? tf : v, bk = k0 + (bnf ? v : tf);
            const float va = A[__mul24(min(m0 + am, M - 1), sam) + __mul24(min(ak, K - 1), sak)];
            const float vb = B[__mul24(min(bk, K - 1), sbk) + __mul24(min(n0 + bn, N - 1), sbn)];
            ra[i] = va;
            rb[i] = vb;
        }
    };
    gload(0);
    for (int k0 = 0; k0 < p.K; k0 += HK) {
        __syncthreads();
#pragma unroll
        for (int i = 0; i < NE; ++i) {
            const int v = tv + 4 * i;
            const float xa = (k0 + (akf ? tf : v) < K) ? ra[i] : 0.f, xb = (k0 + (bnf ? v : tf) < K) ? rb[i] : 0.f;
            *reinterpret_cast<_Float16 *>(Ah + (akf ? v : tf) * HROW + (akf ? tf : v) * 2) = (_Float16)(xa * p.sa);
            *reinterpret_cast<_Float16 *>(Bh + (bnf ? tf : v) * HROW + (bnf ? v : tf) * 2) = (_Float16)(xb * p.sb);
        }
        __syncthreads();
        if (k0 + HK < p.K) gload(k0 + HK);
        const unsigned char *ap = Ah + (wm * 32 + l31) * HROW + hh * 16;
        const unsigned char *bp = Bh + (wn * 32 + l31) * HROW + hh * 16;
#pragma unroll
        for (int ks = 0; ks < HK / 16; ++ks) {
            const f16x8 a = *reinterpret_cast<const f16x8 *>(ap + ks * 32);
            const f16x8 b = *reinterpret_cast<const f16x8 *>(bp + ks * 32);
            acc = __builtin_amdgcn_mfma_f32_32x32x16_f16(a, b, acc, 0, 0, 0);
        }
    }
    const int gn = n0 + wn * 32 + l31;
    if (gn >= p.N) return;
#pragma unroll
    for (int reg = 0; reg < 16; ++reg) {
        const int gm = m0 + wm * 32 + (reg & 3) + 8 * (reg >> 2) + 4 * hh;
        if (gm < p.M) C[(long)gm * p.scm + (long)gn * p.scn] = acc[reg] * p.so;
    }
}

__global__ void __launch_bounds__(256) k_gemm_f32(GemmP p) { gemm_body(p, blockIdx.x, blockIdx.y, blockIdx.z); }
__global__ void __launch_bounds__(256) k_gemm2_f32(GemmP p)
{
    __shared__ __attribute__((aligned(16))) float lds[G2_LDS_FLOATS];
    gemm_body2<2, 2>(p, blockIdx.x, blockIdx.y, blockIdx.z, lds);
}

#define GEMM_MAXP 16
struct GemmGroup {
    int n;
    int h16;
    int shape;
    int tile_start[GEMM_MAXP + 1];
    GemmP prob[GEMM_MAXP];
};

__global__ void __launch_bounds__(256) k_gemm_f32_grouped(const GemmGroup *__restrict__ g)
{
    const int bid = blockIdx.x;
    int pi = 0;
    while (pi + 1 < g->n && bid >= g->tile_start[pi + 1]) ++pi;
    const GemmP p = g->prob[pi];
    const int local = bid - g->tile_start[pi];
    const int tn = (p.N + GT - 1) / GT, tm = (p.M + GT - 1) / GT;
    const int bz = local / (tn * tm), rem = local - bz * tn * tm;
    if (g->h16) gemm_body_h16(p, rem % tn, rem / tn, bz);
    else gemm_body(p, rem % tn, rem / tn, bz);
}

__global__ void __launch_bounds__(256) k_gemm_f32_grouped_linear(const GemmGroup *__restrict__ g, OrnLinearJob job, int gemm_tiles, int lin_blocks,
                                                                 MhPackAll pack, int tile_off)
{
    ORN_PRIO_HIGH();
    extern __shared__ __attribute__((aligned(16))) float lds[];
    if ((int)blockIdx.x >= gemm_tiles + lin_blocks) {
        int layer, pjob;
        const int blk = mh_pack_decode(pack, MH_TAB_T, (int)blockIdx.x - gemm_tiles - lin_blocks, layer, pjob);
        mh_pack_block(pack, layer, pjob, blk, reinterpret_cast<float (*)[65]>(lds));
        return;
    }
    if ((int)blockIdx.x >= gemm_tiles) {
#pragma unroll 1
        for (int r = 0; r < G2_LIN_ROUNDS; ++r)
            orn_linear_silu_wave(job, ((blockIdx.x - gemm_tiles) * G2_LIN_ROUNDS + r) * 4 + (threadIdx.x >> 6), threadIdx.x & 63);
        return;
    }
    const int bid = blockIdx.x + tile_off;
    int pi = 0;
    while (pi + 1 < g->n && bid >= g->tile_start[pi + 1]) ++pi;
    const GemmP p = g->prob[pi];
    const int local = bid - g->tile_start[pi];
    if (g->shape == 1) {
        const int tn = (p.N + 31) / 32, tm = (p.M + 127) / 128;
        const int bz = local / (tn * tm), rem = local - bz * tn * tm;
        gemm_body2<4, 1>(p, rem % tn, rem / tn, bz, lds);
    } else {
        const int tn = (p.N + 63) / 64, tm = (p.M + 63) / 64;
        const int bz = local / (tn * tm), rem = local - bz * tn * tm;
        gemm_body2<2, 2>(p, rem % tn, rem / tn, bz, lds);
    }
}

static void finish_gemm(GemmP &p)
{
    p.a_kfast = (labs(p.sak) <= labs(p.sam)) ? 1 : 0;
    p.b_nfast = (labs(p.sbn) <= labs(p.sbk)) ? 1 : 0;
    p.a_vec = p.sak == 1 ? 1 : 0;
    p.b_vec = p.sbn == 1 ? 1 : 0;
}

static int launch_gemm(GemmP p, int batch, hipStream_t st, const char *name)
{
    finish_gemm(p);
    static const bool old_body = orn_probe_env("ORN_MERGE_OLD_BODY") != nullptr;
    if (p.sbn == 1 && !old_body) hipLaunchKernelGGL(k_gemm2_f32, dim3(orn_cdiv(p.N, GT), orn_cdiv(p.M, GT), batch), dim3(256), 0, st, p);
    else
    hipLaunchKernelGGL(k_gemm_f32, dim3(orn_cdiv(p.N, GT), orn_cdiv(p.M, GT), batch), dim3(256), 0, st, p);
    ORN_LAUNCH_CHECK(name);
    return 0;
}

__global__ void k_bias3(const float *__restrict__ a, const float *__restrict__ b, const float *__restrict__ c, int n,
                        float *__restrict__ out)
{
    const int i = blockIdx.x * blockDim.x + threadIdx.x;
    if (i < n) out[i] = a[i] + (b[i] + c[i]);
}

static GemmP prob_T(const float *w1, const float *w2, int C, int O, float *T)
{
    const int K2 = 2 * C;
    GemmP p = {};
    p.A = w2; p.B = w1; p.C = T;
    p.M = O; p.N = C; p.K = K2;
    p.sam = (long)K2 * 9; p.sak = 9; p.sbk = C; p.sbn = 1; p.scm = (long)C * 9; p.scn = 9;
    p.ba = 1; p.bb = 0; p.bc = 1; p.epi = 0;
    return p;
}
static GemmP prob_T_tapmajor(const float *w1, const float *w2t, int C, int O, float *T)
{
    const int K2 = 2 * C;
    GemmP p = prob_T(w1, w2t, C, O, T);
    p.sam = K2; p.sak = 1; p.ba = (long)O * K2;
    return p;
}
static GemmP prob_S(const float *w3x3, const float *w3x1, const float *w1x3, const float *w3, const float *T, int C, int O,
                    float *wf)
{
    GemmP q = {};
    q.A = w3; q.B = T; q.C = wf;
    q.M = O; q.N = C * 9; q.K = O;
    q.sam = O; q.sak = 1; q.sbk = (long)C * 9; q.sbn = 1; q.scm = (long)C * 9; q.scn = 1;
    q.epi = 1; q.w3x3 = w3x3; q.w1x3 = w1x3; q.w3x1 = w3x1; q.Cch = C;
    return q;
}

int orn_launch_merge_fwd(const float *w3x3, const float *b3x3, const float *w3x1, const float *b3x1,
                         const float *w1x3, const float *b1x3, const float *w1, const float *w2, const float *w3,
                         int C, int O, float *T, float *wf, float *bf, hipStream_t st)
{
    ORN_TRY(launch_gemm(prob_T(w1, w2, C, O, T), 9, st, "merge_T"));
    ORN_TRY(launch_gemm(prob_S(w3x3, w3x1, w1x3, w3, T, C, O, wf), 1, st, "merge_S"));
    hipLaunchKernelGGL(k_bias3, dim3(orn_cdiv(O, 256)), dim3(256), 0, st, b3x3, b1x3, b3x1, O, bf);
    ORN_LAUNCH_CHECK("merge_bias");
    return 0;
}

extern "C" int orn_erb_merge_fwd(const float *w3x3, const float *b3x3, const float *w3x1, const float *b3x1,
                                 const float *w1x3, const float *b1x3, const float *w1, const float *w2,
                                 const float *w3, int C, int O, float *T, float *wf, float *bf, void *stream)
{
    ORN_REQUIRE(w3x3 && b3x3 && w3x1 && b3x1 && w1x3 && b1x3 && w1 && w2 && w3 && T && wf && bf, "erb_merge_fwd: null pointer");
    ORN_REQUIRE(C > 0 && O > 0, "erb_merge_fwd: bad sizes C=%d O=%d", C, O);
    return orn_launch_merge_fwd(w3x3, b3x3, w3x1, b3x1, w1x3, b1x3, w1, w2, w3, C, O, T, wf, bf, (hipStream_t)stream);
}

__global__ void k_merge_bwd_slices(const float *__restrict__ g, const float *__restrict__ dbf, long OC, int O,
                                   float *__restrict__ d3x3, float *__restrict__ db3x3, float *__restrict__ d3x1,
                                   float *__restrict__ db3x1, float *__restrict__ d1x3, float *__restrict__ db1x3)
{
    const long i = (long)blockIdx.x * blockDim.x + threadIdx.x;
    if (i < OC) {
        const float *gg = g + i * 9;
        float v[9];
#pragma unroll
        for (int k = 0; k < 9; ++k) v[k] = gg[k];
        if (d3x3 != g) {
#pragma unroll
            for (int k = 0; k < 9; ++k) d3x3[i * 9 + k] = v[k];
        }
#pragma unroll
        for (int k = 0; k < 3; ++k) {
            d1x3[i * 3 + k] = v[3 + k];
            d3x1[i * 3 + k] = v[3 * k + 1];
        }
    }
    if (i < O) {
        const float d = dbf[i];
        if (db3x3 != dbf) db3x3[i] = d;
        db3x1[i] = d;
        db1x3[i] = d;
    }
}

static GemmP prob_dW3(const float *g, const float *T, int C, int O, float *dw3)
{
    const long n = (long)C * 9;
    GemmP p = {};
    p.A = g; p.B = T; p.C = dw3; p.M = O; p.N = O; p.K = (int)n;
    p.sam = n; p.sak = 1; p.sbk = 1; p.sbn = n; p.scm = O; p.scn = 1;
    return p;
}
static GemmP prob_dT(const float *g, const float *w3, int C, int O, float *dT)
{
    const long n = (long)C * 9;
    GemmP p = {};
    p.A = w3; p.B = g; p.C = dT; p.M = O; p.N = (int)n; p.K = O;
    p.sam = 1; p.sak = O; p.sbk = n; p.sbn = 1; p.scm = n; p.scn = 1;
    return p;
}
static GemmP prob_dW2(const float *dT, const float *w1, int C, int O, float *dw2)
{
    const long n = (long)C * 9;
    const int K2 = 2 * C;
    GemmP p = {};
    p.A = dT; p.B = w1; p.C = dw2; p.M = O; p.N = K2; p.K = C;
    p.sam = n; p.sak = 9; p.sbk = 1; p.sbn = C; p.scm = (long)K2 * 9; p.scn = 9;
    p.ba = 1; p.bb = 0; p.bc = 1;
    return p;
}
static GemmP prob_dW1p(const float *w2, const float *dT, int C, int O, float *dw1p)
{
    const long n = (long)C * 9;
    const int K2 = 2 * C;
    GemmP p = {};
    p.A = w2; p.B = dT; p.C = dw1p; p.M = K2; p.N = C; p.K = O;
    p.sam = 9; p.sak = (long)K2 * 9; p.sbk = n; p.sbn = 9; p.scm = C; p.scn = 1;
    p.ba = 1; p.bb = 1; p.bc = (long)K2 * C;
    return p;
}

extern "C" size_t orn_erb_merge_bwd_ws_bytes(int C, int O)
{
    return orn_align(((size_t)O * C * 9 + 9 * (size_t)2 * C * C) * sizeof(float));
}

int orn_launch_merge_bwd(const float *g, const float *dbf, const float *w1, const float *w2, const float *w3,
                         const float *T, int C, int O, float *d3x3, float *db3x3, float *d3x1, float *db3x1,
                         float *d1x3, float *db1x3, float *dw1, float *dw2, float *dw3, float *ws, hipStream_t st)
{
    const int K2 = 2 * C;
    const long n = (long)C * 9;
    float *dT = ws;
    float *dw1p = ws + (size_t)O * n;
    hipLaunchKernelGGL(k_merge_bwd_slices, dim3(orn_cdiv((long)O * C, 256)), dim3(256), 0, st, g, dbf, (long)O * C, O,
                       d3x3, db3x3, d3x1, db3x1, d1x3, db1x3);
    ORN_LAUNCH_CHECK("merge_bwd_slices");
    ORN_TRY(launch_gemm(prob_dW3(g, T, C, O, dw3), 1, st, "merge_dW3"));
    ORN_TRY(launch_gemm(prob_dT(g, w3, C, O, dT), 1, st, "merge_dT"));
    ORN_TRY(launch_gemm(prob_dW2(dT, w1, C, O, dw2), 9, st, "merge_dW2"));
    ORN_TRY(launch_gemm(prob_dW1p(w2, dT, C, O, dw1p), 9, st, "merge_dW1"));
    ORN_TRY(orn_launch_reduce_rows(dw1p, 9, (size_t)K2 * C, (size_t)K2 * C, dw1, st));
    return 0;
}

extern "C" int orn_erb_merge_bwd(const float *g, const float *dbf, const float *w1, const float *w2, const float *w3,
                                 const float *T, int C, int O, float *d3x3, float *db3x3, float *d3x1, float *db3x1,
                                 float *d1x3, float *db1x3, float *dw1, float *dw2, float *dw3, void *ws,
                                 size_t ws_bytes, void *stream)
{
    ORN_REQUIRE(g && dbf && w1 && w2 && w3 && T && d3x3 && db3x3 && d3x1 && db3x1 && d1x3 && db1x3 && dw1 && dw2 && dw3 && ws,
                "erb_merge_bwd: null pointer");
    ORN_REQUIRE(C > 0 && O > 0, "erb_merge_bwd: bad sizes");
    if (ws_bytes < orn_erb_merge_bwd_ws_bytes(C, O)) {
        orn_set_error("erb_merge_bwd: workspace %zu < %zu", ws_bytes, orn_erb_merge_bwd_ws_bytes(C, O));
        return ORN_E_WS;
    }
    return orn_launch_merge_bwd(g, dbf, w1, w2, w3, T, C, O, d3x3, db3x3, d3x1, db3x1, d1x3, db1x3, dw1, dw2, dw3,
                                (float *)ws, (hipStream_t)stream);
}

#define W2T_ROWS 4
struct W2TAll { int n; int blk_start[ORN_MAX_LAYERS + 1]; struct { const float *w2; float *w2t; int O, K2; } l[ORN_MAX_LAYERS]; };

__global__ void __launch_bounds__(256) k_w2_transpose(W2TAll a, MhPackAll pack, int tr_blocks)
{
    ORN_PRIO_HIGH();
    extern __shared__ float w2s[];
    if ((int)blockIdx.x >= tr_blocks) {
        int layer, pjob;
        const int blk = mh_pack_decode(pack, MH_TAB_PAR, (int)blockIdx.x - tr_blocks, layer, pjob);
        mh_pack_block(pack, layer, pjob, blk, reinterpret_cast<float (*)[65]>(w2s));
        return;
    }
    int li = 0;
    while (li + 1 < a.n && (int)blockIdx.x >= a.blk_start[li + 1]) ++li;
    const auto &l = a.l[li];
    const int m0 = ((int)blockIdx.x - a.blk_start[li]) * W2T_ROWS, rows = min(W2T_ROWS, l.O - m0);
    const int E = l.K2 * 9, t = threadIdx.x;
    const float *src = l.w2 + (size_t)m0 * E;
    const int n = rows * E;
    for (int i0 = t; i0 < n; i0 += 14 * 256) {
        float v[14];
#pragma unroll
        for (int u = 0; u < 14; ++u) v[u] = src[min(i0 + 256 * u, n - 1)];
#pragma unroll
        for (int u = 0; u < 14; ++u)
            if (i0 + 256 * u < n) w2s[i0 + 256 * u] = v[u];
    }
    __syncthreads();
    const int wave = t >> 6, lane = t & 63;
    for (int pb = wave; pb < 9 * rows; pb += 3 * 4) {
        for (int k = lane; k < l.K2; k += 64) {
            float x[3];
#pragma unroll
            for (int a = 0; a < 3; ++a) {
                const int pr = min(pb + 4 * a, 9 * rows - 1), ij = pr / rows, r = pr - ij * rows;
                x[a] = w2s[r * E + ij + k * 9];
            }
#pragma unroll
            for (int a = 0; a < 3; ++a) {
                const int pr = pb + 4 * a;
                if (pr < 9 * rows) {
                    const int ij = pr / rows, r = pr - ij * rows;
                    l.w2t[((size_t)ij * l.O + m0 + r) * l.K2 + k] = x[a];
                }
            }
        }
    }
}

int orn_launch_w2_transpose(int n_layers, const OrnMergeLayer *L, hipStream_t st, const void *pack, int par_blocks)
{
    W2TAll a;
    a.n = 0;
    a.blk_start[0] = 0;
    size_t smem = 0;
    for (int i = 0; i < n_layers; ++i) {
        if (!L[i].w2t) continue;
        auto &l = a.l[a.n];
        l.w2 = L[i].w2; l.w2t = L[i].w2t; l.O = L[i].O; l.K2 = 2 * L[i].C;
        a.blk_start[a.n + 1] = a.blk_start[a.n] + orn_cdiv(l.O, W2T_ROWS);
        const size_t b = (size_t)W2T_ROWS * l.K2 * 9 * sizeof(float);
        if (b > smem) smem = b;
        ++a.n;
    }
    MhPackAll pk = {};
    if (pack && par_blocks > 0) { pk = *(const MhPackAll *)pack; if (smem < 64 * 65 * sizeof(float)) smem = 64 * 65 * sizeof(float); } else par_blocks = 0;
    if (a.n == 0 && par_blocks == 0) return 0;
    ORN_REQUIRE(smem <= 64 * 1024, "w2_transpose: 2C = %zu too wide for the LDS tile", smem / (W2T_ROWS * 9 * sizeof(float)));
    hipLaunchKernelGGL(k_w2_transpose, dim3(a.blk_start[a.n] + par_blocks), dim3(256), smem, st, a, pk, a.blk_start[a.n]);
    ORN_LAUNCH_CHECK("w2_transpose");
    return 0;
}

static void group_add(GemmGroup &g, GemmP p, int batch)
{
    finish_gemm(p);
    const int tiles = (g.shape == 1 ? orn_cdiv(p.N, 32) * orn_cdiv(p.M, 128) : orn_cdiv(p.N, GT) * orn_cdiv(p.M, GT)) * batch;
    g.prob[g.n] = p;
    g.tile_start[g.n + 1] = g.tile_start[g.n] + tiles;
    ++g.n;
}

size_t orn_merge_group_bytes() { return orn_align(4 * sizeof(GemmGroup)); }

int orn_merge_groups_build(void *dev_tables, int n_layers, const OrnMergeLayer *L, int bwd_h16)
{
    ORN_REQUIRE(2 * n_layers <= GEMM_MAXP, "merge groups: too many layers");
    GemmGroup *h = new GemmGroup[4]();
    h[0].shape = 1;
    int s_order[ORN_MAX_LAYERS], n_ord = 0;
    {
        int longest = 0, total = 0;
        for (int i = 0; i < n_layers; ++i) {
            if (L[i].O > L[longest].O) longest = i;
            total += orn_cdiv(L[i].C * 9, GT) * orn_cdiv(L[i].O, GT);
        }
        const int overflow = total > 256 ? total - 256 : 0;
        int cum = 0;
        bool placed = false;
        for (int i = n_layers - 1; i >= 0; --i) {
            if (i == longest) continue;
            if (!placed && cum >= overflow) { s_order[n_ord++] = longest; placed = true; }
            s_order[n_ord++] = i;
            cum += orn_cdiv(L[i].C * 9, GT) * orn_cdiv(L[i].O, GT);
        }
        if (!placed) s_order[n_ord++] = longest;
    }
    for (int j = 0; j < n_layers; ++j) {
        const OrnMergeLayer &l = L[s_order[j]];
        GemmP q = prob_S(l.w3x3, l.w3x1, l.w1x3, l.w3, l.T, l.C, l.O, l.wf);
        q.b3x3 = l.b3x3; q.b1x3 = l.b1x3; q.b3x1 = l.b3x1; q.bf = l.bf;
        if (l.half_kind) { q.half_kind = l.half_kind; q.wb = l.wb; q.wd = l.wd; q.biasp = l.biasp; q.s2 = l.s2; q.Cn = l.O / l.s2; q.Cp = l.Cp; }
        group_add(h[1], q, 1);
    }
    for (int i = 0; i < n_layers; ++i) {
        const OrnMergeLayer &l = L[i];
        group_add(h[0], l.w2t ? prob_T_tapmajor(l.w1, l.w2t, l.C, l.O, l.T) : prob_T(l.w1, l.w2, l.C, l.O, l.T), 9);
        const float GS = 16384.0f;
        GemmP q;
        q = prob_dW3(l.g, l.T, l.C, l.O, l.dw3);   q.sa = GS;   q.sb = 1.0f; q.so = 1.0f / GS; group_add(h[2], q, 1);
        q = prob_dT(l.g, l.w3, l.C, l.O, l.dT);    q.sa = 1.0f; q.sb = GS;   q.so = 1.0f / GS; group_add(h[2], q, 1);
        q = prob_dW2(l.dT, l.w1, l.C, l.O, l.dw2); q.sa = GS;   q.sb = 1.0f; q.so = 1.0f / GS; group_add(h[3], q, 9);
        q = prob_dW1p(l.w2, l.dT, l.C, l.O, l.dw1p); q.sa = 1.0f; q.sb = GS; q.so = 1.0f / GS; group_add(h[3], q, 9);
    }
    h[2].h16 = h[3].h16 = bwd_h16 ? 1 : 0;
    hipError_t e = hipMemcpy(dev_tables, h, 4 * sizeof(GemmGroup), hipMemcpyHostToDevice);
    delete[] h;
    if (e != hipSuccess) { orn_set_error("merge groups: hipMemcpy failed: %s", hipGetErrorString(e)); return (int)e; }
    return 0;
}

int orn_merge_group_tiles(int which, int n_layers, const OrnMergeLayer *L)
{
    int t = 0;
    for (int i = 0; i < n_layers; ++i) {
        const int C = L[i].C, O = L[i].O, n = C * 9, K2 = 2 * C;
        switch (which) {
        case 0: t += orn_cdiv(C, 32) * orn_cdiv(O, 128) * 9; break;
        case 1: t += orn_cdiv(n, GT) * orn_cdiv(O, GT); break;
        case 2: t += orn_cdiv(O, GT) * orn_cdiv(O, GT) + orn_cdiv(n, GT) * orn_cdiv(O, GT); break;
        default: t += orn_cdiv(K2, GT) * orn_cdiv(O, GT) * 9 + orn_cdiv(C, GT) * orn_cdiv(K2, GT) * 9; break;
        }
    }
    return t;
}

int orn_launch_merge_group(const void *dev_tables, int which, int tiles, hipStream_t st)
{
    const GemmGroup *g = (const GemmGroup *)dev_tables + which;
    hipLaunchKernelGGL(k_gemm_f32_grouped, dim3(tiles), dim3(256), 0, st, g);
    ORN_LAUNCH_CHECK("merge_group");
    return 0;
}

int orn_launch_merge_group_linear(const void *dev_tables, int which, int tiles, const OrnLinearJob &job, hipStream_t st, const void *pack,
                                  int pack_blocks)
{
    const GemmGroup *g = (const GemmGroup *)dev_tables + which;
    int lin_blocks = orn_cdiv(job.N, 4 * G2_LIN_ROUNDS);
    const size_t smem = G2_LDS_BYTES(which == 0 ? 1 : 0) > 64 * 65 * 4 ? G2_LDS_BYTES(which == 0 ? 1 : 0) : 64 * 65 * 4;
    MhPackAll pk = {};
    if (pack && pack_blocks > 0) pk = *(const MhPackAll *)pack; else pack_blocks = 0;
#ifdef ORN_PROBE_BUILD
    static const int dbg = orn_probe_env_int("ORN_MERGE_DBG", 0);
#else
    constexpr int dbg = 0;
#endif
    if (dbg & 1) pack_blocks = 0;
    if (dbg & 2) lin_blocks = 0;
    if (dbg & 4) {
        GemmGroup hg;
        if (hipMemcpy(&hg, g, sizeof(hg), hipMemcpyDeviceToHost) != hipSuccess) return ORN_E_ARG;
        for (int i = 0; i < hg.n; ++i) {
            const int nt = hg.tile_start[i + 1] - hg.tile_start[i];
            hipLaunchKernelGGL(k_gemm_f32_grouped_linear, dim3(nt), dim3(256), smem, st, g, job, nt, 0, pk, hg.tile_start[i]);
        }
        ORN_LAUNCH_CHECK("merge_group_linear(dbg)");
        return 0;
    }
    hipLaunchKernelGGL(k_gemm_f32_grouped_linear, dim3(tiles + lin_blocks + pack_blocks), dim3(256), smem, st, g, job, tiles, lin_blocks, pk, 0);
    ORN_LAUNCH_CHECK("merge_group_linear");
    return 0;
}

int orn_launch_merge_bias(const float *b3x3, const float *b1x3, const float *b3x1, int O, float *bf, hipStream_t st)
{
    hipLaunchKernelGGL(k_bias3, dim3(orn_cdiv(O, 256)), dim3(256), 0, st, b3x3, b1x3, b3x1, O, bf);
    ORN_LAUNCH_CHECK("merge_bias");
    return 0;
}

int orn_launch_merge_bwd_tail(const float *g, const float *dbf, int C, int O, float *d3x3, float *db3x3, float *d3x1,
                              float *db3x1, float *d1x3, float *db1x3, const float *dw1p, float *dw1, hipStream_t st)
{
    hipLaunchKernelGGL(k_merge_bwd_slices, dim3(orn_cdiv((long)O * C, 256)), dim3(256), 0, st, g, dbf, (long)O * C, O, d3x3,
                       db3x3, d3x1, db3x1, d1x3, db1x3);
    ORN_LAUNCH_CHECK("merge_bwd_slices");
    return orn_launch_reduce_rows(dw1p, 9, (size_t)2 * C * C, (size_t)2 * C * C, dw1, st);
}

struct MiscLayers {
    int n;
    OrnMergeMisc l[ORN_MAX_LAYERS];
};

__global__ void k_merge_bias_all(MiscLayers m)
{
    const OrnMergeMisc &l = m.l[blockIdx.y];
    const int i = blockIdx.x * blockDim.x + threadIdx.x;
    if (i < l.O) l.bf[i] = l.b3x3[i] + (l.b1x3[i] + l.b3x1[i]);
}

__global__ void k_merge_bwd_tail_all(MiscLayers m)
{
    ORN_PRIO_HIGH();
    const OrnMergeMisc &l = m.l[blockIdx.y];
    const long i = (long)blockIdx.x * blockDim.x + threadIdx.x;
    const long OC = (long)l.O * l.C;
    if (i < OC) {
        const float *gg = l.g + i * 9;
#pragma unroll
        for (int k = 0; k < 3; ++k) {
            l.d1x3[i * 3 + k] = gg[3 + k];
            l.d3x1[i * 3 + k] = gg[3 * k + 1];
        }
    }
    if (i < l.O) {
        const float d = l.dbf[i];
        l.db3x1[i] = d;
        l.db1x3[i] = d;
    }
    const long n1 = (long)2 * l.C * l.C;
    if (i < n1) {
        float acc = 0.f;
#pragma unroll
        for (int k = 0; k < 9; ++k) acc += l.dw1p[(long)k * n1 + i];
        l.dw1[i] = acc;
    }
    if (l.dw2t) {
        const long n2 = (long)l.O * 2 * l.C;
        for (long j = i; j < n2; j += (long)gridDim.x * blockDim.x) {
            float v[9];
#pragma unroll
            for (int k = 0; k < 9; ++k) v[k] = l.dw2t[(long)k * n2 + j];
#pragma unroll
            for (int k = 0; k < 9; ++k) l.dw2[j * 9 + k] = v[k];
        }
    }
}

int orn_launch_merge_bias_all(int n, const OrnMergeMisc *L, hipStream_t st)
{
    MiscLayers m;
    m.n = n;
    int maxO = 0;
    for (int i = 0; i < n; ++i) { m.l[i] = L[i]; if (L[i].O > maxO) maxO = L[i].O; }
    hipLaunchKernelGGL(k_merge_bias_all, dim3(orn_cdiv(maxO, 256), n), dim3(256), 0, st, m);
    ORN_LAUNCH_CHECK("merge_bias_all");
    return 0;
}

int orn_launch_merge_bwd_tail_all(int n, const OrnMergeMisc *L, hipStream_t st)
{
    MiscLayers m;
    m.n = n;
    long mx = 0;
    for (int i = 0; i < n; ++i) {
        m.l[i] = L[i];
        const long w = (long)L[i].O * L[i].C > (long)2 * L[i].C * L[i].C ? (long)L[i].O * L[i].C : (long)2 * L[i].C * L[i].C;
        if (w > mx) mx = w;
    }
    hipLaunchKernelGGL(k_merge_bwd_tail_all, dim3(orn_cdiv(mx, 256), n), dim3(256), 0, st, m);
    ORN_LAUNCH_CHECK("merge_bwd_tail_all");
    return 0;
}
```

boosting-neural-video-representation-via-online-structural-reparameteration_amd/csrc/orn_merge_h16.hip:

```cpp
#include "orn_internal.h"
#include "orn_merge_pack.h"
#include <new>

typedef __attribute__((ext_vector_type(8))) _Float16 mh16x8;
typedef __attribute__((ext_vector_type(16))) float mf32x16;


struct MhSizes { size_t gh, gt, th, w3t, w1h, w2p, dtt, dtc; };
static MhSizes mh_sizes(int C, int O)
{
    const int E = 9 * C, K2 = 2 * C;
    MhSizes s;
    s.gh = (size_t)r32(O) * r16(E);
    s.gt = (size_t)r32(E) * r16(O);
    s.th = (size_t)r32(O) * r16(E);
    s.w3t = (size_t)r32(O) * r16(O);
    s.w1h = (size_t)r32(K2) * r16(C);
    s.w2p = (size_t)9 * r32(K2) * r16(O);
    s.dtt = (size_t)9 * r32(O) * r16(C);
    s.dtc = (size_t)9 * r32(C) * r16(O);
    return s;
}

size_t orn_merge_h16_layer_halfs(int C, int O)
{
    const MhSizes s = mh_sizes(C, O);
    const size_t parts[8] = {s.gh, s.gt, s.th, s.w3t, s.w1h, s.w2p, s.dtt, s.dtc};
    size_t tot = 0;
    for (int i = 0; i < 8; ++i) tot += (parts[i] + 127) / 128 * 128;
    return tot;
}

__global__ void __launch_bounds__(256) k_merge_pack(MhPackAll a, int fwd )
{
    ORN_PRIO_HIGH();
    __shared__ float tile[64][65];
    int layer, job;
    const int blk = mh_pack_decode(a, fwd, (int)blockIdx.x, layer, job);
    mh_pack_block(a, layer, job, blk, tile);
}

struct MhProb {
    const mh16 *A, *B;
    int lda, ldb, M, N, K;
    long ba, bb;
    int nbatch;
    int mode;
    float *C; long scm, scn, bc; float so;
    mh16 *dtt, *dtc; int Cch, ldt, ldc; long st_t, st_c;
    int tiles_n, tiles;
};
#define MH_MAXP 16
#define MH_KB 8
struct MhGroup { int n; int tile_start[MH_MAXP + 1]; MhProb p[MH_MAXP]; };

__global__ void __launch_bounds__(256) k_mgemm_h16(const MhGroup *__restrict__ g, int total_tiles, OrnScaleState *sc)
{
    ORN_PRIO_HIGH();
    __shared__ float part[4][16][64];
    const int wave = __builtin_amdgcn_readfirstlane(threadIdx.x >> 6);
    const int lane = threadIdx.x & 63, l31 = lane & 31, hh = lane >> 5;
    const int tile = blockIdx.x;
    int pi = 0;
    while (pi + 1 < g->n && tile >= g->tile_start[pi + 1]) ++pi;
    const MhProb &p = g->p[pi];
    const int local = tile - g->tile_start[pi];
    const int b = local / p.tiles, r = local - b * p.tiles;
    const int tm = r / p.tiles_n, tn = r - tm * p.tiles_n;
    const int nsteps = p.K / 16, per = (nsteps + 3) / 4;
    const int s0 = min(wave * per, nsteps), s1 = min(s0 + per, nsteps);
    const mh16 *ap = p.A + (size_t)b * p.ba + (size_t)(tm * 32 + l31) * p.lda + hh * 8 + s0 * 16;
    const mh16 *bp = p.B + (size_t)b * p.bb + (size_t)(tn * 32 + l31) * p.ldb + hh * 8 + s0 * 16;
    mf32x16 acc;
#pragma unroll
    for (int i = 0; i < 16; ++i) acc[i] = 0.f;
    const int K = (s1 - s0) * 16;
    int k = 0;
    mh16x8 fa[MH_KB], fb[MH_KB];
    constexpr int KD = MH_KB * 16;
    if (K >= KD) {
#pragma unroll
        for (int j = 0; j < MH_KB; ++j) { fa[j] = *reinterpret_cast<const mh16x8 *>(ap + j * 16); fb[j] = *reinterpret_cast<const mh16x8 *>(bp + j * 16); }
        for (k = KD; k + KD <= K; k += KD) {
            mh16x8 na[MH_KB], nb[MH_KB];
#pragma unroll
            for (int j = 0; j < MH_KB; ++j) { na[j] = *reinterpret_cast<const mh16x8 *>(ap + k + j * 16); nb[j] = *reinterpret_cast<const mh16x8 *>(bp + k + j * 16); }
#pragma unroll
            for (int j = 0; j < MH_KB; ++j) acc = __builtin_amdgcn_mfma_f32_32x32x16_f16(fa[j], fb[j], acc, 0, 0, 0);
#pragma unroll
            for (int j = 0; j < MH_KB; ++j) { fa[j] = na[j]; fb[j] = nb[j]; }
        }
        mh16x8 ta[MH_KB], tb[MH_KB];
        const int nt = (K - k) / 16;
#pragma unroll
        for (int j = 0; j < MH_KB; ++j)
            if (j < nt) { ta[j] = *reinterpret_cast<const mh16x8 *>(ap + k + j * 16); tb[j] = *reinterpret_cast<const mh16x8 *>(bp + k + j * 16); }
#pragma unroll
        for (int j = 0; j < MH_KB; ++j) acc = __builtin_amdgcn_mfma_f32_32x32x16_f16(fa[j], fb[j], acc, 0, 0, 0);
#pragma unroll
        for (int j = 0; j < MH_KB; ++j)
            if (j < nt) acc = __builtin_amdgcn_mfma_f32_32x32x16_f16(ta[j], tb[j], acc, 0, 0, 0);
        k = K;
    }
    if (k < K) {
        mh16x8 ta[MH_KB], tb[MH_KB];
        const int nt = (K - k) / 16;
#pragma unroll
        for (int j = 0; j < MH_KB; ++j)
            if (j < nt) { ta[j] = *reinterpret_cast<const mh16x8 *>(ap + k + j * 16); tb[j] = *reinterpret_cast<const mh16x8 *>(bp + k + j * 16); }
#pragma unroll
        for (int j = 0; j < MH_KB; ++j)
            if (j < nt) acc = __builtin_amdgcn_mfma_f32_32x32x16_f16(ta[j], tb[j], acc, 0, 0, 0);
    }
#pragma unroll
    for (int i = 0; i < 16; ++i) part[wave][i][lane] = acc[i];
    __syncthreads();
    float sum[4];
#pragma unroll
    for (int i = 0; i < 4; ++i) {
        const int reg = 4 * wave + i;
        sum[i] = ((part[0][reg][lane] + part[1][reg][lane]) + part[2][reg][lane]) + part[3][reg][lane];
    }
    const int n = tn * 32 + l31;
    if (n >= p.N) return;
    if (p.mode == 0) {
        float *C = p.C + (size_t)b * p.bc + (size_t)n * p.scn;
#pragma unroll
        for (int i = 0; i < 4; ++i) {
            const int reg = 4 * wave + i, m = tm * 32 + (reg & 3) + 8 * (reg >> 2) + 4 * hh;
            if (m < p.M) C[(size_t)m * p.scm] = sum[i] * p.so;
        }
    } else {
        const int c = n / 9, ij = n - c * 9;
        mh16 *t = p.dtt + (size_t)ij * p.st_t + c;
        mh16 *u = p.dtc + (size_t)ij * p.st_c + (size_t)c * p.ldc;
        bool bad = false;
#pragma unroll
        for (int i = 0; i < 4; ++i) {
            const int reg = 4 * wave + i, m = tm * 32 + (reg & 3) + 8 * (reg >> 2) + 4 * hh;
            if (m < p.M) {
                const mh16 v = (mh16)sum[i];
                t[(size_t)m * p.ldt] = v;
                u[m] = v;
                bad |= !(fabsf((float)v) <= 3.0e38f);
            }
        }
        if (bad) orn_flag_nonfinite(sc, __builtin_nanf(""));
    }
}

struct OrnMergeH16 {
    MhPackAll pack;
    int pack_blocks_grad, pack_blocks_par, pack_blocks_t;
    int tiles[2];
};

static void mh_add(MhGroup &g, MhProb p)
{
    p.tiles_n = (p.N + 31) / 32;
    p.tiles = ((p.M + 31) / 32) * p.tiles_n;
    g.p[g.n] = p;
    g.tile_start[g.n + 1] = g.tile_start[g.n] + p.tiles * p.nbatch;
    ++g.n;
}

size_t orn_merge_h16_table_bytes() { return orn_align(2 * sizeof(MhGroup)); }
size_t orn_merge_h16_host_bytes() { return sizeof(OrnMergeH16); }

int orn_merge_h16_build(void *dev_tables, void *host, int n_layers, const OrnMergeLayer *L, void *const *bufs, OrnScaleState *sc)
{
    ORN_REQUIRE(2 * n_layers <= MH_MAXP && n_layers <= ORN_MAX_LAYERS, "merge h16: too many layers");
    OrnMergeH16 *H = new (host) OrnMergeH16();
    MhGroup *G = new MhGroup[2]();
    H->pack.n = n_layers;
    H->pack.sc = sc;
    H->pack.grad_start[0] = 0;
    H->pack.par_start[0] = 0;
    H->pack.tt_start[0] = 0;
    for (int i = 0; i < n_layers; ++i) {
        const OrnMergeLayer &l = L[i];
        const int C = l.C, O = l.O, E = 9 * C, K2 = 2 * C;
        const MhSizes s = mh_sizes(C, O);
        mh16 *base = (mh16 *)bufs[i];
        auto take = [&](size_t n) { mh16 *p = base; base += (n + 127) / 128 * 128; return p; };
        mh16 *gh = take(s.gh), *gt = take(s.gt), *th = take(s.th), *w3t = take(s.w3t), *w1h = take(s.w1h), *w2p = take(s.w2p);
        mh16 *dtt = take(s.dtt), *dtc = take(s.dtc);
        H->pack.l[i] = MhPackLayer{C, O, l.g, l.T, l.w1, l.w2, l.w3, gh, gt, th, w3t, w1h, w2p};
        const int jobs[MH_JOBS] = {orn_cdiv((long)O * E, 256 * MH_CPT), orn_cdiv((long)O * E, 256 * MH_CPT), orn_cdiv((long)K2 * C, 256 * MH_CPT),
                                   orn_cdiv(O, 64) * orn_cdiv(E, 64), orn_cdiv(O, 64) * orn_cdiv(O, 64), orn_cdiv(O, 64) * orn_cdiv(K2 * 9, 64)};
        H->pack.grad_start[2 * i + 1] = H->pack.grad_start[2 * i] + jobs[0];
        H->pack.grad_start[2 * i + 2] = H->pack.grad_start[2 * i + 1] + jobs[3];
        const int pj[3] = {jobs[2], jobs[4], jobs[5]};
        for (int j = 0; j < 3; ++j) H->pack.par_start[3 * i + j + 1] = H->pack.par_start[3 * i + j] + pj[j];
        H->pack.tt_start[i + 1] = H->pack.tt_start[i] + jobs[1];
        MhProb p;
        p = MhProb{};
        p.A = gh; p.lda = r16(E); p.B = th; p.ldb = r16(E); p.M = O; p.N = O; p.K = r16(E); p.nbatch = 1;
        p.mode = 0; p.C = l.dw3; p.scm = O; p.scn = 1; p.so = 1.0f / MH_GS;
        mh_add(G[0], p);
        p = MhProb{};
        p.A = w3t; p.lda = r16(O); p.B = gt; p.ldb = r16(O); p.M = O; p.N = E; p.K = r16(O); p.nbatch = 1;
        p.mode = 1; p.dtt = dtt; p.dtc = dtc; p.Cch = C; p.ldt = r16(C); p.ldc = r16(O);
        p.st_t = (long)r32(O) * r16(C); p.st_c = (long)r32(C) * r16(O);
        mh_add(G[0], p);
        p = MhProb{};
        p.A = dtt; p.lda = r16(C); p.ba = (long)r32(O) * r16(C); p.B = w1h; p.ldb = r16(C); p.bb = 0;
        p.M = O; p.N = K2; p.K = r16(C); p.nbatch = 9;
        p.mode = 0; p.C = l.dw2t; p.scm = K2; p.scn = 1; p.bc = (long)O * K2; p.so = 1.0f / MH_GS;
        mh_add(G[1], p);
        p = MhProb{};
        p.A = w2p; p.lda = r16(O); p.ba = (long)r32(K2) * r16(O); p.B = dtc; p.ldb = r16(O); p.bb = (long)r32(C) * r16(O);
        p.M = K2; p.N = C; p.K = r16(O); p.nbatch = 9;
        p.mode = 0; p.C = l.dw1p; p.scm = C; p.scn = 1; p.bc = (long)K2 * C; p.so = 1.0f / MH_GS;
        mh_add(G[1], p);
    }
    H->pack_blocks_grad = H->pack.grad_start[2 * n_layers];
    H->pack_blocks_par = H->pack.par_start[3 * n_layers];
    H->pack_blocks_t = H->pack.tt_start[n_layers];
    H->tiles[0] = G[0].tile_start[G[0].n];
    H->tiles[1] = G[1].tile_start[G[1].n];
    hipError_t e = hipMemcpy(dev_tables, G, 2 * sizeof(MhGroup), hipMemcpyHostToDevice);
    delete[] G;
    if (e != hipSuccess) { orn_set_error("merge h16: hipMemcpy failed: %s", hipGetErrorString(e)); return (int)e; }
    return 0;
}

const void *orn_merge_h16_pack(const void *host, int *par_blocks, int *t_blocks)
{
    const OrnMergeH16 *H = (const OrnMergeH16 *)host;
    *par_blocks = H->pack_blocks_par;
    *t_blocks = H->pack_blocks_t;
    return &H->pack;
}

int orn_launch_merge_h16_pack_jobs(const void *host, int which, hipStream_t st)
{
    const OrnMergeH16 *H = (const OrnMergeH16 *)host;
    const int blocks = which == MH_TAB_PAR ? H->pack_blocks_par : H->pack_blocks_t;
    if (blocks <= 0) return 0;
    hipLaunchKernelGGL(k_merge_pack, dim3(blocks), dim3(256), 0, st, H->pack, which);
    ORN_LAUNCH_CHECK("merge_pack(jobs)");
    return 0;
}

int orn_launch_merge_h16_bwd(const void *dev_tables, const void *host, hipStream_t st, OrnScaleState *sc)
{
    const OrnMergeH16 *H = (const OrnMergeH16 *)host;
    MhPackAll pack = H->pack;
    if (sc) pack.sc = sc;
    hipLaunchKernelGGL(k_merge_pack, dim3(H->pack_blocks_grad), dim3(256), 0, st, pack, (int)MH_TAB_GRAD);
    ORN_LAUNCH_CHECK("merge_pack");
    const MhGroup *g = (const MhGroup *)dev_tables;
    hipLaunchKernelGGL(k_mgemm_h16, dim3(H->tiles[0]), dim3(256), 0, st, g, H->tiles[0], pack.sc);
    ORN_LAUNCH_CHECK("mgemm_h16(dW3,dT)");
    hipLaunchKernelGGL(k_mgemm_h16, dim3(H->tiles[1]), dim3(256), 0, st, g + 1, H->tiles[1], (OrnScaleState *)nullptr);
    ORN_LAUNCH_CHECK("mgemm_h16(dW2,dW1)");
    return 0;
}

extern "C" int orn_debug_merge_h16_bwd(int n, const int *co, const float *const *in, float *const *out, int *flag, void *stream)
{
    ORN_REQUIRE(n >= 1 && n <= ORN_MAX_LAYERS && co && in && out && flag, "debug_merge_h16_bwd: bad arguments");
    for (int i = 0; i < n; ++i) ORN_REQUIRE(co[2 * i] >= 1 && co[2 * i + 1] >= 1, "debug_merge_h16_bwd: layer %d: C, O >= 1", i);
    hipStream_t st = (hipStream_t)stream;
    const size_t a0 = 256, a1 = a0 + orn_align(orn_merge_h16_table_bytes());
    size_t off[ORN_MAX_LAYERS][3], tot = a1;
    for (int i = 0; i < n; ++i) {
        const size_t C = co[2 * i], O = co[2 * i + 1];
        off[i][0] = tot; tot += orn_align(orn_merge_h16_layer_halfs((int)C, (int)O) * 2);
        off[i][1] = tot; tot += orn_align(9 * O * 2 * C * 4);
        off[i][2] = tot; tot += orn_align(9 * 2 * C * C * 4);
    }
    char *ws = nullptr;
    ORN_HIP(hipMalloc(&ws, tot));
    void *host = malloc(orn_merge_h16_host_bytes());
    int rc = host ? 0 : ORN_E_ARG;
    OrnScaleState *sc = (OrnScaleState *)ws;
    OrnMergeLayer L[ORN_MAX_LAYERS] = {};
    OrnMergeMisc M[ORN_MAX_LAYERS] = {};
    void *bufs[ORN_MAX_LAYERS];
    for (int i = 0; i < n; ++i) {
        const float *const *p = in + 6 * i;
        float *const *q = out + 7 * i;
        OrnMergeLayer &l = L[i];
        l.C = co[2 * i]; l.O = co[2 * i + 1];
        l.g = p[0]; l.T = const_cast<float *>(p[2]); l.w1 = p[3]; l.w2 = p[4]; l.w3 = p[5];
        l.dw3 = q[0]; l.dw2 = q[1]; l.dw2t = (float *)(ws + off[i][1]); l.dw1p = (float *)(ws + off[i][2]);
        bufs[i] = ws + off[i][0];
        M[i] = OrnMergeMisc{};
        M[i].C = l.C; M[i].O = l.O; M[i].g = l.g; M[i].dbf = p[1]; M[i].dw1p = l.dw1p;
        M[i].dw1 = q[2]; M[i].d1x3 = q[3]; M[i].d3x1 = q[4]; M[i].db1x3 = q[5]; M[i].db3x1 = q[6];
        M[i].dw2t = l.dw2t; M[i].dw2 = q[1];
    }
    OrnScaleState s0 = {};
    s0.gs = s0.inv_gs = s0.gs_max = 1.0f;
    hipError_t e = hipSuccess;
    if (rc == 0 && (e = hipMemset(ws, 0, tot)) == hipSuccess) e = hipMemcpy(sc, &s0, sizeof(s0), hipMemcpyHostToDevice);
    if (rc == 0 && e != hipSuccess) { orn_set_error("debug_merge_h16_bwd: %s", hipGetErrorString(e)); rc = (int)e; }
    if (rc == 0) rc = orn_merge_h16_build(ws + a0, host, n, L, bufs, sc);
    if (rc == 0) rc = orn_launch_merge_h16_pack_jobs(host, MH_TAB_PAR, st);
    if (rc == 0) rc = orn_launch_merge_h16_pack_jobs(host, MH_TAB_T, st);
    if (rc == 0) rc = orn_launch_merge_h16_bwd(ws + a0, host, st, sc);
    if (rc == 0) rc = orn_launch_merge_bwd_tail_all(n, M, st);
    if (rc == 0 && (e = hipStreamSynchronize(st)) == hipSuccess) e = hipMemcpy(&s0, sc, sizeof(s0), hipMemcpyDeviceToHost);
    if (rc == 0 && e != hipSuccess) { orn_set_error("debug_merge_h16_bwd: %s", hipGetErrorString(e)); rc = (int)e; }
    if (rc == 0) *flag = s0.flag;
    free(host);
    (void)hipFree(ws);
    return rc;
}
```

boosting-neural-video-representation-via-online-structural-reparameteration_amd/csrc/orn_wgrad_bf16.hip:

```cpp
#include "orn_h16.h"

namespace HNS {

#include "orn_wgrad_body.h"
static int g_wgrad_dbg = 0;
void set_debug_wgrad(int flags) { g_wgrad_dbg = flags; }

__global__ void __launch_bounds__(256, 2) k_wgrad_nhwc_bf16(WgradBP p) { wgrad_body(p, blockIdx.x); }

__device__ __forceinline__ void head_finish_body(const float *__restrict__ partial, int blocks, int C, float gscale, float *__restrict__ dw,
                                                 float *__restrict__ db, int col, float *sred , OrnScaleState *sc = nullptr)
{
    if (sc) gscale = sc->inv_gs;
    const int n = 3 * C + 3, t = threadIdx.x;
    float acc = 0.f;
    for (int r = t; r < blocks; r += 256) acc += partial[(size_t)r * n + col];
    sred[t] = acc;
    __syncthreads();
    for (int w = 128; w > 0; w >>= 1) {
        if (t < w) sred[t] += sred[t + w];
        __syncthreads();
    }
    if (t == 0) {
        const float v = sred[0] * gscale;
        orn_flag_nonfinite(sc, v);
        if (col < 3 * C) dw[col] = v;
        else db[col - 3 * C] = v;
    }
}

__global__ void __launch_bounds__(256) k_head_bf16_finish(const float *__restrict__ partial, int blocks, int C, float gscale,
                                                          float *__restrict__ dw, float *__restrict__ db)
{
    __shared__ float sred[256];
    head_finish_body(partial, blocks, C, gscale, dw, db, blockIdx.x, sred);
}

int orn_launch_head_finish_bf16(const float *partial, int blocks, int C, float gscale, float *dw, float *db, hipStream_t st)
{
    hipLaunchKernelGGL(k_head_bf16_finish, dim3(3 * C + 3), dim3(256), 0, st, partial, blocks, C, gscale, dw, db);
    ORN_LAUNCH_CHECK("head_bf16_finish");
    return 0;
}

struct WgradBPAll { int n; int start[ORN_MAX_LAYERS + 1]; WgradBP p[ORN_MAX_LAYERS]; OrnHeadFinish hf; int hf_blocks; OrnStemL2Job l2; int side; };
__global__ void __launch_bounds__(256, 2) k_wgrad_nhwc_bf16_all(WgradBPAll a)
{
    if (!a.side) ORN_PRIO_HIGH();
    if ((int)blockIdx.x >= a.start[a.n] + a.hf_blocks) {
        extern __shared__ __attribute__((aligned(16))) unsigned char smem_l2[];
        orn_stem_l2_block(a.l2, (int)blockIdx.x - a.start[a.n] - a.hf_blocks, (int)threadIdx.x, reinterpret_cast<float *>(smem_l2));
        return;
    }
    if ((int)blockIdx.x >= a.start[a.n]) {
        extern __shared__ __attribute__((aligned(16))) unsigned char smem_hf[];
        head_finish_body(a.hf.partial, a.hf.blocks, a.hf.C, a.hf.gscale, a.hf.dw, a.hf.db, (int)blockIdx.x - a.start[a.n],
                         reinterpret_cast<float *>(smem_hf), a.hf.sc);
        return;
    }
    int k = 0;
    while (k + 1 < a.n && (int)blockIdx.x >= a.start[k + 1]) ++k;
    k = __builtin_amdgcn_readfirstlane(k);
    wgrad_body(a.p[k], (int)blockIdx.x - a.start[k]);
}

__device__ __forceinline__ void wgrad_reduce_body(const float *__restrict__ slabs, const float *__restrict__ bias_slabs, int S, int O, int Cn,
                                                  int s2, int Cr, float gscale, float *__restrict__ dwf, float *__restrict__ dbf,
                                                  OrnScaleState *sc = nullptr)
{
    if (sc) gscale = sc->inv_gs;
    const size_t n = (size_t)9 * O * 96;
    const size_t idx = (size_t)blockIdx.x * blockDim.x + threadIdx.x;
    if (idx < (size_t)O && dbf) {
        float b = 0.f;
        for (int s = 0; s < S; ++s) b += bias_slabs[(size_t)s * O + idx];
        const int ij = (int)idx / Cn, nn = (int)idx - ij * Cn;
        dbf[nn * s2 + ij] = b * gscale;
        orn_flag_nonfinite(sc, b * gscale);
    }
    if (idx >= n) return;
    const int c = (int)(idx % 96);
    if (c >= Cr) return;
    float a8[8] = {0.f, 0.f, 0.f, 0.f, 0.f, 0.f, 0.f, 0.f};
    int s = 0;
    for (; s + 8 <= S; s += 8) {
#pragma unroll
        for (int k = 0; k < 8; ++k) a8[k] += slabs[(size_t)(s + k) * n + idx];
    }
    for (; s < S; ++s) a8[0] += slabs[(size_t)s * n + idx];
    const float acc = ((a8[0] + a8[1]) + (a8[2] + a8[3])) + ((a8[4] + a8[5]) + (a8[6] + a8[7]));
    const size_t r = idx / 96;
    const int op = (int)(r % O), tap = (int)(r / O);
    const int ij = op / Cn, nn = op - ij * Cn;
    const int o = nn * s2 + ij;
    dwf[((size_t)o * Cr + c) * 9 + tap] = acc * gscale;
    orn_flag_nonfinite(sc, acc * gscale);
}

__global__ void k_wgrad_bf16_reduce(const float *__restrict__ slabs, const float *__restrict__ bias_slabs, int S, int O, int Cn,
                                    int s2, int Cr, float gscale, float *__restrict__ dwf, float *__restrict__ dbf)
{
    wgrad_reduce_body(slabs, bias_slabs, S, O, Cn, s2, Cr, gscale, dwf, dbf);
}

struct WgradReduceAll {
    struct { const float *slabs, *bias_slabs; int S, O, Cn, s2, Cr; float gscale; float *dwf, *dbf; OrnScaleState *sc; } l[ORN_MAX_LAYERS];
    int n; OrnStemW0Job w0;
};
__global__ void k_wgrad_bf16_reduce_all(WgradReduceAll a)
{
    if ((int)blockIdx.y == a.n) {
        __shared__ float sh_w0[4];
        if (2 * (int)blockIdx.x >= a.w0.N) return;
        const int half = threadIdx.x >> 7;
        orn_stem_w0_row(a.w0, (int)blockIdx.x * 2 + half, threadIdx.x & 127, sh_w0 + 2 * half);
        return;
    }
    const auto &l = a.l[blockIdx.y];
    if ((size_t)blockIdx.x * blockDim.x >= (size_t)9 * l.O * 96) return;
    wgrad_reduce_body(l.slabs, l.bias_slabs, l.S, l.O, l.Cn, l.s2, l.Cr, l.gscale, l.dwf, l.dbf, l.sc);
}

int orn_wgrad_bf16_split(int H, int W, int O, int smax = 0)
{
    const int n_ktiles = orn_cdiv(H, WB_TH) * orn_cdiv(W, WB_TW);
    const int per = 3 * orn_cdiv(O, WB_BO);
    int S = (512 / per) / 8 * 8;
    static const int s_env = orn_probe_env_int("ORN_WGRAD_SMAX", 0);
    if (s_env > 0 && S > s_env) S = s_env;
    if (S > 40) S = 40;
    static const int s_small = orn_probe_env_int("ORN_WGRAD_SMAX_SMALL", 24);
    if (n_ktiles < 2000 && S > s_small && smax < 8) S = s_small;
    const int by_work = (n_ktiles / 8) / 8 * 8;
    if (S > by_work) S = by_work;
    if (smax >= 8 && S > smax) S = smax / 8 * 8;
    if (S < 8) S = 8;
    return S;
}

size_t orn_wgrad_bf16_ws_floats(int H, int W, int O)
{
    const int S = orn_wgrad_bf16_split(H, W, O), Smax = orn_wgrad_bf16_split(H, W, O, 40);
    return (size_t)(S > Smax ? S : Smax) * (9 * (size_t)O * 96 + O);
}

static int wgrad_fill(WgradBP &p, const h16 *xpad, const h16 *dypad, int H, int W, int C, int O, int s, float *slabs, int smax = 0)
{
    ORN_REQUIRE(C >= 1 && C <= 96 && O % 32 == 0 && O % (s * s) == 0, "wgrad_bf16: unsupported C=%d O=%d", C, O);
    p.dbg = g_wgrad_dbg;
    p.xpad = xpad; p.dypad = dypad; p.slabs = slabs; p.H = H; p.W = W; p.O = O;
    p.tiles_w = orn_cdiv(W, WB_TW);
    p.n_ktiles = p.tiles_w * orn_cdiv(H, WB_TH);
    p.S = orn_wgrad_bf16_split(H, W, O, smax);
    p.bias_slabs = slabs + (size_t)p.S * 9 * O * 96;
    p.n_otiles = orn_cdiv(O, WB_BO);
    static bool attr_done = false;
    if (!attr_done) {
        const size_t smem = WB_LDS_BYTES;
        hipError_t e = hipFuncSetAttribute((const void *)k_wgrad_nhwc_bf16, hipFuncAttributeMaxDynamicSharedMemorySize, (int)smem);
        if (e == hipSuccess) e = hipFuncSetAttribute((const void *)k_wgrad_nhwc_bf16_all, hipFuncAttributeMaxDynamicSharedMemorySize, (int)smem);
        if (e != hipSuccess) { orn_set_error("wgrad_bf16: hipFuncSetAttribute: %s", hipGetErrorString(e)); return (int)e; }
        attr_done = true;
    }
    return 0;
}

int orn_launch_wgrad_bf16_batch(int n, const OrnWgradJob *J, hipStream_t st, const OrnHeadFinish *hf, const OrnStemL2Job *l2, int side)
{
    if (n == 0 && !hf && !l2) return 0;
    ORN_REQUIRE(n <= ORN_MAX_LAYERS, "wgrad_batch: %d layers", n);
    WgradBPAll a;
    a.n = n;
    a.side = side;
    int total = 0;
    for (int i = 0; i < n; ++i) {
        ORN_TRY(wgrad_fill(a.p[i], (const h16 *)J[i].xpad, (const h16 *)J[i].dypad, J[i].H, J[i].W, J[i].C, J[i].O, J[i].s, J[i].slabs, J[i].smax));
        a.start[i] = total;
        total += 3 * a.p[i].n_otiles * a.p[i].S;
    }
    a.start[n] = total;
    a.hf = OrnHeadFinish{};
    a.hf_blocks = 0;
    if (hf) { a.hf = *hf; a.hf_blocks = 3 * hf->C + 3; total += a.hf_blocks; }
    a.l2 = OrnStemL2Job{};
    if (l2) { a.l2 = *l2; total += orn_cdiv(l2->N, ORN_STEM_ROWS); }
    hipLaunchKernelGGL(k_wgrad_nhwc_bf16_all, dim3(total), dim3(256), WB_LDS_BYTES, st, a);
    ORN_LAUNCH_CHECK("wgrad_nhwc_bf16_all");
    return 0;
}

int orn_launch_wgrad_bf16(const h16 *xpad, const h16 *dypad, int H, int W, int C, int O, int s, float gscale,
                          float *slabs, float *dwf, float *dbf, hipStream_t st)
{
    WgradBP p;
    ORN_TRY(wgrad_fill(p, xpad, dypad, H, W, C, O, s, slabs));
    hipLaunchKernelGGL(k_wgrad_nhwc_bf16, dim3(3 * p.n_otiles * p.S), dim3(256), WB_LDS_BYTES, st, p);
    ORN_LAUNCH_CHECK("wgrad_nhwc_bf16");
    if (!dwf) return 0;
    const size_t n = (size_t)9 * O * 96;
    hipLaunchKernelGGL(k_wgrad_bf16_reduce, dim3(orn_cdiv((long)n, 256)), dim3(256), 0, st, slabs, p.bias_slabs, p.S, O,
                       O / (s * s), s * s, C, gscale, dwf, dbf);
    ORN_LAUNCH_CHECK("wgrad_bf16_reduce");
    return 0;
}

int orn_launch_wgrad_reduce_all(int n, const OrnWgradReduce *L, hipStream_t st, const OrnStemW0Job *w0)
{
    if (n == 0 && !w0) return 0;
    ORN_REQUIRE(n <= ORN_MAX_LAYERS, "wgrad_reduce_all: %d layers", n);
    WgradReduceAll a;
    size_t mx = 0;
    for (int i = 0; i < n; ++i) {
        const int S = orn_wgrad_bf16_split(L[i].H, L[i].W, L[i].O, L[i].smax), s2 = L[i].s * L[i].s;
        a.l[i].slabs = L[i].slabs; a.l[i].bias_slabs = L[i].slabs + (size_t)S * 9 * L[i].O * 96;
        a.l[i].S = S; a.l[i].O = L[i].O; a.l[i].Cn = L[i].O / s2; a.l[i].s2 = s2; a.l[i].Cr = L[i].C; a.l[i].gscale = L[i].gscale;
        a.l[i].dwf = L[i].dwf; a.l[i].dbf = L[i].dbf; a.l[i].sc = L[i].sc;
        const size_t w = (size_t)9 * L[i].O * 96;
        if (w > mx) mx = w;
    }
    a.n = n;
    a.w0 = OrnStemW0Job{};
    if (w0) { a.w0 = *w0; const size_t need = (size_t)orn_cdiv(w0->N, 2) * 256; if (need > mx) mx = need; }
    hipLaunchKernelGGL(k_wgrad_bf16_reduce_all, dim3(orn_cdiv((long)mx, 256), n + (w0 ? 1 : 0)), dim3(256), 0, st, a);
    ORN_LAUNCH_CHECK("wgrad_bf16_reduce_all");
    return 0;
}

}
```

include/orn_debug.h:

```cpp
#ifndef ORN_DEBUG_H_
#define ORN_DEBUG_H_
#include "orn.h"
#ifdef __cplusplus
extern "C" {
#endif
ORN_API void orn_debug_set(int flags);
ORN_API int orn_debug_conv_fwd_bf16(const void *xpad, const void *wb, const float *bias_p, int H, int W, int Cin, int O, int s,
                                    void *z, void *apad, int c_real, void *stream);
ORN_API int orn_debug_conv_fwd_f16(const void *xpad, const void *wb, const float *bias_p, int H, int W, int Cin, int O, int s,
                                   void *z, void *apad, int c_real, void *stream);
ORN_API int orn_debug_conv_dgrad_bf16(const void *dypad, const void *wd, int H, int W, int O, int C, const void *zprev,
                                      void *dyprev, int sp, float *dx_f32, int c_real, void *stream);
ORN_API int orn_debug_conv_dgrad_f16(const void *dypad, const void *wd, int H, int W, int O, int C, const void *zprev,
                                     void *dyprev, int sp, float *dx_f32, int c_real, void *stream);
ORN_API int orn_debug_merge_h16_bwd(int n, const int *co, const float *const *in, float *const *out, int *flag, void *stream);
ORN_API size_t orn_debug_decode_out_ws_bytes(void);
ORN_API int orn_debug_decode_out_f32(const float *img, int H, int W, const float *target, uint8_t *rgb8, float *img_out,
                                     float *stats, void *ws, size_t ws_bytes, void *stream);
#ifdef ORN_CONV_STAMP
ORN_API void orn_debug_set_stamps(void *buf);
#endif
#ifdef __cplusplus
}
#endif
#endif
```

Measured before the change: 1024 frames/s.

## Drop w2 transpose pass via tap-strided T GEMM and fuse grad packing into wgrad reduce

Result: no change. 1023 frames/s (-0.1%).

```diff
diff --git a/boosting-neural-video-representation-via-online-structural-reparameteration_amd/csrc/orn_engine.hip b/boosting-neural-video-representation-via-online-structural-reparameteration_amd/csrc/orn_engine.hip
--- a/boosting-neural-video-representation-via-online-structural-reparameteration_amd/csrc/orn_engine.hip
+++ b/boosting-neural-video-representation-via-online-structural-reparameteration_amd/csrc/orn_engine.hip
@@ -5,7 +5,6 @@
 
 struct LayerBuf {
     float *T, *wf, *bf;
-    float *w2t;
     float *dT, *dw1p;
     float *wd32;
     void *mh16;
@@ -153,7 +152,6 @@
         const size_t wsz = (size_t)l.O * l.C * 9;
         if (d->erb) {
             L[i].T = take(wsz); L[i].wf = take(wsz); L[i].bf = take(l.O);
-            L[i].w2t = (2 * l.C * 9 * 4 * 4 <= 64 * 1024) ? take((size_t)9 * l.O * 2 * l.C) : nullptr;
             L[i].dT = take(wsz); L[i].dw1p = take((size_t)9 * 2 * l.C * l.C);
             if (d->precision != 0) {
                 L[i].mh16 = take((orn_merge_h16_layer_halfs(l.C, l.O) + 1) / 2);
@@ -310,7 +308,7 @@
             m.C = l.C; m.O = l.O;
             m.w3x3 = params + l.w3x3; m.w3x1 = params + l.w3x1; m.w1x3 = params + l.w1x3;
             m.w1 = params + l.w1; m.w2 = params + l.w2; m.w3 = params + l.w3;
-            m.T = e->L[i].T; m.wf = e->L[i].wf; m.w2t = e->L[i].w2t;
+            m.T = e->L[i].T; m.wf = e->L[i].wf;
             m.b3x3 = params + l.b3x3; m.b1x3 = params + l.b1x3; m.b3x1 = params + l.b3x1; m.bf = e->L[i].bf;
             m.g = grads ? grads + l.w3x3 : nullptr;
             m.dT = e->L[i].dT; m.dw1p = e->L[i].dw1p;
@@ -407,6 +405,16 @@
     return 0;
 }
 
+extern "C" int orn_debug_engine_grad_halfs(orn_engine *e, int layer, const void **gh, const void **gt, int *ldh, int *ldt)
+{
+    ORN_REQUIRE(e && gh && gt && ldh && ldt && layer >= 0 && layer < e->d.n_layers, "debug_engine_grad_halfs: bad arguments");
+    ORN_REQUIRE(e->d.erb && e->mset[0].mh_host, "debug_engine_grad_halfs: no 16-bit ERB engine");
+    void *h, *t;
+    orn_merge_h16_grad_halfs(e->mset[0].mh_host, layer, &h, &t, ldh, ldt);
+    *gh = h; *gt = t;
+    return 0;
+}
+
 extern "C" int orn_engine_fused_kernel(orn_engine *e, int layer, const float **wf, const float **bf)
 {
     ORN_REQUIRE(e && wf && bf && layer >= 0 && layer < e->d.n_layers, "engine_fused_kernel: bad arguments");
@@ -478,7 +486,7 @@
 static OrnWgradReduce wgrad_reduce(const orn_engine *e, int i, OrnScaleState *sc)
 {
     const orn_layer_desc &l = e->d.layer[i];
-    return OrnWgradReduce{e->L[i].wslab, l.H, l.W, l.C, l.O, l.s, 1.0f / e->gs, e->grads + l.w3x3, e->grads + l.b3x3, sc, slab_cap(e, i)};
+    return OrnWgradReduce{e->L[i].wslab, l.H, l.W, l.C, l.O, l.s, 1.0f / e->gs, e->grads + l.w3x3, e->grads + l.b3x3, sc, slab_cap(e, i), nullptr, nullptr, 0, 0};
 }
 
 enum { MERGE_NONE = -1 };
@@ -498,8 +506,7 @@
         const orn_engine::MergeSet &ms = e->mset[set];
         int pk_par = 0, pk_t = 0;
         const void *pk = (keep_z && ms.mh_host) ? orn_merge_h16_pack(ms.mh_host, &pk_par, &pk_t) : nullptr;
-        ORN_TRY(orn_launch_w2_transpose(ms.n, ms.ml, st, pk, pk_par));
-        ORN_TRY(orn_launch_merge_group_linear(ms.tables, 0, ms.tiles[0], lin1, st));
+        ORN_TRY(orn_launch_merge_group_linear(ms.tables, 0, ms.tiles[0], lin1, st, pk, pk_par));
         ORN_TRY(orn_launch_merge_group_linear(ms.tables, 1, ms.tiles[1], lin2, st, e->stage0 ? nullptr : pk, e->stage0 ? 0 : pk_t));
         pack_t = e->stage0 ? pk : nullptr; pack_t_blocks = e->stage0 ? pk_t : 0;
     } else {
@@ -624,11 +631,12 @@
     const OrnHeadFinish hf = {e->head_ws, e->ops->head_bwd_blocks(e->Hout, e->Wout), e->Cn_last, 1.0f / e->gs, G + d.head_w, G + d.head_b, sc};
     ORN_TRY(e->ops->wgrad_batch(1, &wj, sd, &hf, nullptr, 1));
     ORN_HIP(hipEventRecord(e->ev_wgrad, sd));
-    const OrnWgradReduce wr = wgrad_reduce(e, nl - 1, sc);
+    OrnWgradReduce wr = wgrad_reduce(e, nl - 1, sc);
+    if (d.erb) orn_merge_h16_grad_halfs(e->mset[2].mh_host, 0, &wr.gh, &wr.gt, &wr.ldh, &wr.ldt);
     ORN_TRY(e->ops->wgrad_reduce_all(1, &wr, sd, nullptr));
     if (d.erb) {
         const orn_engine::MergeSet &ms = e->mset[2];
-        ORN_TRY(orn_launch_merge_h16_bwd(ms.mh_tables, ms.mh_host, sd, sc));
+        ORN_TRY(orn_launch_merge_h16_bwd(ms.mh_tables, ms.mh_host, sd, sc, true));
         const OrnMergeMisc mm = merge_misc(e, nl - 1);
         ORN_TRY(orn_launch_merge_bwd_tail_all(1, &mm, sd));
     }
@@ -648,7 +656,6 @@
     if (more && d.erb) {
         const orn_engine::MergeSet &ms = e->mset[2];
         const OrnLinearJob none = {};
-        ORN_TRY(orn_launch_w2_transpose(ms.n, ms.ml, sd));
         ORN_TRY(orn_launch_merge_group_linear(ms.tables, 0, ms.tiles[0], none, sd));
         ORN_TRY(orn_launch_merge_group_linear(ms.tables, 1, ms.tiles[1], none, sd));
         packs = ms.mh_host;
diff --git a/boosting-neural-video-representation-via-online-structural-reparameteration_amd/csrc/orn_internal.h b/boosting-neural-video-representation-via-online-structural-reparameteration_amd/csrc/orn_internal.h
--- a/boosting-neural-video-representation-via-online-structural-reparameteration_amd/csrc/orn_internal.h
+++ b/boosting-neural-video-representation-via-online-structural-reparameteration_amd/csrc/orn_internal.h
@@ -43,7 +43,6 @@
     const float *w3x3, *w3x1, *w1x3, *w1, *w2, *w3;
     const float *b3x3, *b1x3, *b3x1; float *bf;
     float *T, *wf;
-    float *w2t;
     const float *g;
     float *dT, *dw1p, *dw2, *dw3;
     float *dw2t;
@@ -52,7 +51,6 @@
     float *biasp;
 };
 size_t orn_merge_group_bytes();
-int orn_launch_w2_transpose(int n_layers, const OrnMergeLayer *L, hipStream_t st, const void *pack = nullptr, int par_blocks = 0);
 int orn_merge_groups_build(void *dev_tables, int n_layers, const OrnMergeLayer *L, int bwd_h16);
 int orn_merge_group_tiles(int which, int n_layers, const OrnMergeLayer *L);
 int orn_launch_merge_group(const void *dev_tables, int which, int tiles, hipStream_t st);
@@ -66,7 +64,9 @@
 size_t orn_merge_h16_table_bytes();
 size_t orn_merge_h16_host_bytes();
 int orn_merge_h16_build(void *dev_tables, void *host, int n_layers, const OrnMergeLayer *L, void *const *bufs, OrnScaleState *sc);
-int orn_launch_merge_h16_bwd(const void *dev_tables, const void *host, hipStream_t st, OrnScaleState *sc = nullptr);
+int orn_launch_merge_h16_bwd(const void *dev_tables, const void *host, hipStream_t st, OrnScaleState *sc = nullptr,
+                             bool packed = false);
+void orn_merge_h16_grad_halfs(const void *host, int i, void **gh, void **gt, int *ldh, int *ldt);
 const void *orn_merge_h16_pack(const void *host, int *par_blocks, int *t_blocks);
 int orn_launch_merge_h16_pack_jobs(const void *host, int which, hipStream_t st);
 
@@ -99,7 +99,8 @@
                     OrnLossFinalJob *defer = nullptr);
 
 struct OrnPrepLayer { const float *wf, *bf; int O, C, s; void *wb, *wd; float *biasp; int Cp; };
-struct OrnWgradReduce { const float *slabs; int H, W, C, O, s; float gscale; float *dwf, *dbf; OrnScaleState *sc; int smax; };
+struct OrnWgradReduce { const float *slabs; int H, W, C, O, s; float gscale; float *dwf, *dbf; OrnScaleState *sc; int smax;
+                        void *gh, *gt; int ldh, ldt; };
 struct OrnHeadFinish { const float *partial; int blocks, C; float gscale; float *dw, *db; OrnScaleState *sc; };
 struct OrnWgradJob { const void *xpad, *dypad; int H, W, C, O, s; float *slabs; int smax; };
 struct OrnHeadFuse { const float *w, *b; float *out; int sigmoid; int fused; };
diff --git a/boosting-neural-video-representation-via-online-structural-reparameteration_amd/csrc/orn_merge.hip b/boosting-neural-video-representation-via-online-structural-reparameteration_amd/csrc/orn_merge.hip
--- a/boosting-neural-video-representation-via-online-structural-reparameteration_amd/csrc/orn_merge.hip
+++ b/boosting-neural-video-representation-via-online-structural-reparameteration_amd/csrc/orn_merge.hip
@@ -13,6 +13,7 @@
     long ba, bb, bc;
     int a_kfast, b_nfast;
     int a_vec, b_vec;
+    int t_vec;
     int epi;
     const float *w3x3, *w1x3, *w3x1;
     int Cch;
@@ -359,9 +360,109 @@
     }
 #endif
 }
-#define G2_LDS_FLOATS (3 * (128 * G2_KC + G2_KC * 32))
-#define G2_LDS_BYTES(shape_) ((shape_) == 1 ? 3 * (128 * G2_KC + G2_KC * 32) * 4 : 3 * (64 * G2_KC + G2_KC * 64) * 4)
+#define G2_LDS_FLOATS (3 * (64 * G2_KC + G2_KC * 64))
+#define G2_LDS_BYTES (G2_LDS_FLOATS * 4)
 #define G2_LIN_ROUNDS 4
+
+#define GT_KC 32
+#define GT_LDA (9 * GT_KC + 4)
+#define GT_LDS_FLOATS (32 * GT_LDA + GT_KC * 32)
+#define GT_LDS_BYTES (GT_LDS_FLOATS * 4)
+template <bool TVEC>
+__device__ __forceinline__ void gemm_body_tv(const GemmP &p, int tg, int bx, int by, float *lds)
+{
+    constexpr int UPR = 9 * GT_KC / 4;
+    constexpr int NU = 32 * UPR / 256;
+    static_assert(32 * UPR % 256 == 0, "whole units per thread");
+    float *As = lds, *Bs = lds + 32 * GT_LDA;
+    const int t = threadIdx.x, lane = t & 63, wave = __builtin_amdgcn_readfirstlane(t >> 6);
+    const int l31 = lane & 31, hh = lane >> 5;
+    const int m0 = by * 32, n0 = bx * 32;
+    const int M = p.M, N = p.N, K = p.K;
+    const unsigned run = (unsigned)p.sam, sbk = (unsigned)p.sbk;
+    const unsigned a_bytes = (unsigned)M * run * 4u;
+    const unsigned b_bytes = ((unsigned)(K - 1) * sbk + (unsigned)N) * 4u;
+    const auto rA = __builtin_amdgcn_make_buffer_rsrc(const_cast<float *>(p.A), 0, a_bytes, 0x00020000);
+    const auto rB = __builtin_amdgcn_make_buffer_rsrc(const_cast<float *>(p.B), 0, b_bytes, 0x00020000);
+    struct Regs { float4 a[NU]; float4 b; };
+    unsigned a_vo[NU];
+    int a_dst[NU];
+#pragma unroll
+    for (int i = 0; i < NU; ++i) {
+        const int v = t + 256 * i, row = v / UPR, u = v - row * UPR;
+        a_vo[i] = ((unsigned)(m0 + row) * run + 4u * (unsigned)u) * 4u;
+        a_dst[i] = row * GT_LDA + 4 * u;
+    }
+    const unsigned b_vo = ((unsigned)(t >> 3) * sbk + (unsigned)(n0 + 4 * (t & 7))) * 4u;
+    const int b_dst = (t >> 3) * 32 + 4 * (t & 7);
+    const int nreal = (K + GT_KC - 1) / GT_KC;
+    constexpr unsigned BEYOND = 0x80000000u;
+    auto gload = [&](Regs &R, int c) {
+        const bool live = c < nreal;
+        const unsigned so = live ? (unsigned)c * (GT_KC * 9 * 4u) : 0u;
+#pragma unroll
+        for (int i = 0; i < NU; ++i) {
+            const unsigned vo = live ? a_vo[i] : BEYOND;
+            if constexpr (TVEC) R.a[i] = G2_LOAD16(rA, vo, so);
+            else {
+                R.a[i].x = __builtin_bit_cast(float, __builtin_amdgcn_raw_buffer_load_b32(rA, vo, so, 0));
+                R.a[i].y = __builtin_bit_cast(float, __builtin_amdgcn_raw_buffer_load_b32(rA, vo + 4u, so, 0));
+                R.a[i].z = __builtin_bit_cast(float, __builtin_amdgcn_raw_buffer_load_b32(rA, vo + 8u, so, 0));
+                R.a[i].w = __builtin_bit_cast(float, __builtin_amdgcn_raw_buffer_load_b32(rA, vo + 12u, so, 0));
+            }
+        }
+        R.b = G2_LOAD16(rB, live ? b_vo : BEYOND, live ? (unsigned)c * (GT_KC * 4u) * sbk : 0u);
+    };
+    auto lstore = [&](const Regs &R) {
+#pragma unroll
+        for (int i = 0; i < NU; ++i) *reinterpret_cast<float4 *>(As + a_dst[i]) = R.a[i];
+        *reinterpret_cast<float4 *>(Bs + b_dst) = R.b;
+    };
+    f32x16 acc;
+#pragma unroll
+    for (int r = 0; r < 16; ++r) acc[r] = 0.f;
+    const int tap = 3 * tg + wave;
+    const float *ap = As + l31 * GT_LDA + 9 * hh + tap, *bp = Bs + hh * 32 + l31;
+    auto step = [&](Regs &R, int c) {
+        __syncthreads();
+        lstore(R);
+        __syncthreads();
+        gload(R, c + 3);
+        if (wave < 3) {
+#pragma unroll
+            for (int s = 0; s < GT_KC / 2; ++s)
+                acc = __builtin_amdgcn_mfma_f32_32x32x2f32(ap[18 * s], bp[64 * s], acc, 0, 0, 0);
+        }
+    };
+    Regs R0, R1, R2;
+    gload(R0, 0);
+    gload(R1, 1);
+    gload(R2, 2);
+    const int nch = (nreal + 2) / 3 * 3;
+    for (int c = 0; c < nch; c += 3) {
+        step(R0, c);
+        step(R1, c + 1);
+        step(R2, c + 2);
+    }
+    const int gn = n0 + l31;
+    if (wave < 3 && gn < N) {
+        float *C = p.C + tap;
+#pragma unroll
+        for (int reg = 0; reg < 16; ++reg) {
+            const int gm = m0 + (reg & 3) + 8 * (reg >> 2) + 4 * hh;
+            if (gm < M) C[(long)gm * p.scm + (long)gn * p.scn] = acc[reg];
+        }
+    }
+}
+__device__ __forceinline__ void gemm_body_t(const GemmP &p, int local, float *lds)
+{
+    const int tn = (p.N + 31) / 32;
+    const int tg = local % 3, r = local / 3;
+    if (p.t_vec) gemm_body_tv<true>(p, tg, r % tn, r / tn, lds);
+    else gemm_body_tv<false>(p, tg, r % tn, r / tn, lds);
+}
+static inline int gemm_t_tiles(int M, int N) { return 3 * orn_cdiv(N, 32) * orn_cdiv(M, 32); }
+
 template <int WM, int WN>
 __device__ __forceinline__ void gemm_body2(const GemmP &p, int bx, int by, int bz, float *lds)
 {
@@ -442,6 +543,12 @@
     gemm_body2<2, 2>(p, blockIdx.x, blockIdx.y, blockIdx.z, lds);
 }
 
+__global__ void __launch_bounds__(256) k_gemm_t_f32(GemmP p)
+{
+    extern __shared__ __attribute__((aligned(16))) float lds_t[];
+    gemm_body_t(p, blockIdx.x, lds_t);
+}
+
 #define GEMM_MAXP 16
 struct GemmGroup {
     int n;
@@ -465,13 +572,13 @@
 }
 
 __global__ void __launch_bounds__(256) k_gemm_f32_grouped_linear(const GemmGroup *__restrict__ g, OrnLinearJob job, int gemm_tiles, int lin_blocks,
-                                                                 MhPackAll pack, int tile_off)
+                                                                 MhPackAll pack, int pack_tab, int tile_off)
 {
     ORN_PRIO_HIGH();
     extern __shared__ __attribute__((aligned(16))) float lds[];
     if ((int)blockIdx.x >= gemm_tiles + lin_blocks) {
         int layer, pjob;
-        const int blk = mh_pack_decode(pack, MH_TAB_T, (int)blockIdx.x - gemm_tiles - lin_blocks, layer, pjob);
+        const int blk = mh_pack_decode(pack, pack_tab, (int)blockIdx.x - gemm_tiles - lin_blocks, layer, pjob);
         mh_pack_block(pack, layer, pjob, blk, reinterpret_cast<float (*)[65]>(lds));
         return;
     }
@@ -487,9 +594,7 @@
     const GemmP p = g->prob[pi];
     const int local = bid - g->tile_start[pi];
     if (g->shape == 1) {
-        const int tn = (p.N + 31) / 32, tm = (p.M + 127) / 128;
-        const int bz = local / (tn * tm), rem = local - bz * tn * tm;
-        gemm_body2<4, 1>(p, rem % tn, rem / tn, bz, lds);
+        gemm_body_t(p, local, lds);
     } else {
         const int tn = (p.N + 63) / 64, tm = (p.M + 63) / 64;
         const int bz = local / (tn * tm), rem = local - bz * tn * tm;
@@ -503,6 +608,7 @@
     p.b_nfast = (labs(p.sbn) <= labs(p.sbk)) ? 1 : 0;
     p.a_vec = p.sak == 1 ? 1 : 0;
     p.b_vec = p.sbn == 1 ? 1 : 0;
+    p.t_vec = (p.sam % 4 == 0 && (uintptr_t)p.A % 16 == 0) ? 1 : 0;
 }
 
 static int launch_gemm(GemmP p, int batch, hipStream_t st, const char *name)
@@ -533,13 +639,6 @@
     p.ba = 1; p.bb = 0; p.bc = 1; p.epi = 0;
     return p;
 }
-static GemmP prob_T_tapmajor(const float *w1, const float *w2t, int C, int O, float *T)
-{
-    const int K2 = 2 * C;
-    GemmP p = prob_T(w1, w2t, C, O, T);
-    p.sam = K2; p.sak = 1; p.ba = (long)O * K2;
-    return p;
-}
 static GemmP prob_S(const float *w3x3, const float *w3x1, const float *w1x3, const float *w3, const float *T, int C, int O,
                     float *wf)
 {
@@ -555,7 +654,10 @@
                          const float *w1x3, const float *b1x3, const float *w1, const float *w2, const float *w3,
                          int C, int O, float *T, float *wf, float *bf, hipStream_t st)
 {
-    ORN_TRY(launch_gemm(prob_T(w1, w2, C, O, T), 9, st, "merge_T"));
+    GemmP pt = prob_T(w1, w2, C, O, T);
+    finish_gemm(pt);
+    hipLaunchKernelGGL(k_gemm_t_f32, dim3(gemm_t_tiles(pt.M, pt.N)), dim3(256), GT_LDS_BYTES, st, pt);
+    ORN_LAUNCH_CHECK("merge_T");
     ORN_TRY(launch_gemm(prob_S(w3x3, w3x1, w1x3, w3, T, C, O, wf), 1, st, "merge_S"));
     hipLaunchKernelGGL(k_bias3, dim3(orn_cdiv(O, 256)), dim3(256), 0, st, b3x3, b1x3, b3x1, O, bf);
     ORN_LAUNCH_CHECK("merge_bias");
@@ -676,84 +778,10 @@
                                 (float *)ws, (hipStream_t)stream);
 }
 
-#define W2T_ROWS 4
-struct W2TAll { int n; int blk_start[ORN_MAX_LAYERS + 1]; struct { const float *w2; float *w2t; int O, K2; } l[ORN_MAX_LAYERS]; };
-
-__global__ void __launch_bounds__(256) k_w2_transpose(W2TAll a, MhPackAll pack, int tr_blocks)
-{
-    ORN_PRIO_HIGH();
-    extern __shared__ float w2s[];
-    if ((int)blockIdx.x >= tr_blocks) {
-        int layer, pjob;
-        const int blk = mh_pack_decode(pack, MH_TAB_PAR, (int)blockIdx.x - tr_blocks, layer, pjob);
-        mh_pack_block(pack, layer, pjob, blk, reinterpret_cast<float (*)[65]>(w2s));
-        return;
-    }
-    int li = 0;
-    while (li + 1 < a.n && (int)blockIdx.x >= a.blk_start[li + 1]) ++li;
-    const auto &l = a.l[li];
-    const int m0 = ((int)blockIdx.x - a.blk_start[li]) * W2T_ROWS, rows = min(W2T_ROWS, l.O - m0);
-    const int E = l.K2 * 9, t = threadIdx.x;
-    const float *src = l.w2 + (size_t)m0 * E;
-    const int n = rows * E;
-    for (int i0 = t; i0 < n; i0 += 14 * 256) {
-        float v[14];
-#pragma unroll
-        for (int u = 0; u < 14; ++u) v[u] = src[min(i0 + 256 * u, n - 1)];
-#pragma unroll
-        for (int u = 0; u < 14; ++u)
-            if (i0 + 256 * u < n) w2s[i0 + 256 * u] = v[u];
-    }
-    __syncthreads();
-    const int wave = t >> 6, lane = t & 63;
-    for (int pb = wave; pb < 9 * rows; pb += 3 * 4) {
-        for (int k = lane; k < l.K2; k += 64) {
-            float x[3];
-#pragma unroll
-            for (int a = 0; a < 3; ++a) {
-                const int pr = min(pb + 4 * a, 9 * rows - 1), ij = pr / rows, r = pr - ij * rows;
-                x[a] = w2s[r * E + ij + k * 9];
-            }
-#pragma unroll
-            for (int a = 0; a < 3; ++a) {
-                const int pr = pb + 4 * a;
-                if (pr < 9 * rows) {
-                    const int ij = pr / rows, r = pr - ij * rows;
-                    l.w2t[((size_t)ij * l.O + m0 + r) * l.K2 + k] = x[a];
-                }
-            }
-        }
-    }
-}
-
-int orn_launch_w2_transpose(int n_layers, const OrnMergeLayer *L, hipStream_t st, const void *pack, int par_blocks)
-{
-    W2TAll a;
-    a.n = 0;
-    a.blk_start[0] = 0;
-    size_t smem = 0;
-    for (int i = 0; i < n_layers; ++i) {
-        if (!L[i].w2t) continue;
-        auto &l = a.l[a.n];
-        l.w2 = L[i].w2; l.w2t = L[i].w2t; l.O = L[i].O; l.K2 = 2 * L[i].C;
-        a.blk_start[a.n + 1] = a.blk_start[a.n] + orn_cdiv(l.O, W2T_ROWS);
-        const size_t b = (size_t)W2T_ROWS * l.K2 * 9 * sizeof(float);
-        if (b > smem) smem = b;
-        ++a.n;
-    }
-    MhPackAll pk = {};
-    if (pack && par_blocks > 0) { pk = *(const MhPackAll *)pack; if (smem < 64 * 65 * sizeof(float)) smem = 64 * 65 * sizeof(float); } else par_blocks = 0;
-    if (a.n == 0 && par_blocks == 0) return 0;
-    ORN_REQUIRE(smem <= 64 * 1024, "w2_transpose: 2C = %zu too wide for the LDS tile", smem / (W2T_ROWS * 9 * sizeof(float)));
-    hipLaunchKernelGGL(k_w2_transpose, dim3(a.blk_start[a.n] + par_blocks), dim3(256), smem, st, a, pk, a.blk_start[a.n]);
-    ORN_LAUNCH_CHECK("w2_transpose");
-    return 0;
-}
-
 static void group_add(GemmGroup &g, GemmP p, int batch)
 {
     finish_gemm(p);
-    const int tiles = (g.shape == 1 ? orn_cdiv(p.N, 32) * orn_cdiv(p.M, 128) : orn_cdiv(p.N, GT) * orn_cdiv(p.M, GT)) * batch;
+    const int tiles = g.shape == 1 ? gemm_t_tiles(p.M, p.N) : orn_cdiv(p.N, GT) * orn_cdiv(p.M, GT) * batch;
     g.prob[g.n] = p;
     g.tile_start[g.n + 1] = g.tile_start[g.n] + tiles;
     ++g.n;
@@ -793,7 +821,7 @@
     }
     for (int i = 0; i < n_layers; ++i) {
         const OrnMergeLayer &l = L[i];
-        group_add(h[0], l.w2t ? prob_T_tapmajor(l.w1, l.w2t, l.C, l.O, l.T) : prob_T(l.w1, l.w2, l.C, l.O, l.T), 9);
+        group_add(h[0], prob_T(l.w1, l.w2, l.C, l.O, l.T), 1);
         const float GS = 16384.0f;
         GemmP q;
         q = prob_dW3(l.g, l.T, l.C, l.O, l.dw3);   q.sa = GS;   q.sb = 1.0f; q.so = 1.0f / GS; group_add(h[2], q, 1);
@@ -814,7 +842,7 @@
     for (int i = 0; i < n_layers; ++i) {
         const int C = L[i].C, O = L[i].O, n = C * 9, K2 = 2 * C;
         switch (which) {
-        case 0: t += orn_cdiv(C, 32) * orn_cdiv(O, 128) * 9; break;
+        case 0: t += gemm_t_tiles(O, C); break;
         case 1: t += orn_cdiv(n, GT) * orn_cdiv(O, GT); break;
         case 2: t += orn_cdiv(O, GT) * orn_cdiv(O, GT) + orn_cdiv(n, GT) * orn_cdiv(O, GT); break;
         default: t += orn_cdiv(K2, GT) * orn_cdiv(O, GT) * 9 + orn_cdiv(C, GT) * orn_cdiv(K2, GT) * 9; break;
@@ -836,7 +864,9 @@
 {
     const GemmGroup *g = (const GemmGroup *)dev_tables + which;
     int lin_blocks = orn_cdiv(job.N, 4 * G2_LIN_ROUNDS);
-    const size_t smem = G2_LDS_BYTES(which == 0 ? 1 : 0) > 64 * 65 * 4 ? G2_LDS_BYTES(which == 0 ? 1 : 0) : 64 * 65 * 4;
+    const size_t smem = which == 0 ? GT_LDS_BYTES : G2_LDS_BYTES;
+    static_assert(GT_LDS_BYTES >= 64 * 65 * 4 && G2_LDS_BYTES >= 64 * 65 * 4, "the riders' transpose tile");
+    const int pack_tab = which == 0 ? MH_TAB_PAR : MH_TAB_T;
     MhPackAll pk = {};
     if (pack && pack_blocks > 0) pk = *(const MhPackAll *)pack; else pack_blocks = 0;
 #ifdef ORN_PROBE_BUILD
@@ -851,12 +881,12 @@
         if (hipMemcpy(&hg, g, sizeof(hg), hipMemcpyDeviceToHost) != hipSuccess) return ORN_E_ARG;
         for (int i = 0; i < hg.n; ++i) {
             const int nt = hg.tile_start[i + 1] - hg.tile_start[i];
-            hipLaunchKernelGGL(k_gemm_f32_grouped_linear, dim3(nt), dim3(256), smem, st, g, job, nt, 0, pk, hg.tile_start[i]);
+            hipLaunchKernelGGL(k_gemm_f32_grouped_linear, dim3(nt), dim3(256), smem, st, g, job, nt, 0, pk, pack_tab, hg.tile_start[i]);
         }
         ORN_LAUNCH_CHECK("merge_group_linear(dbg)");
         return 0;
     }
-    hipLaunchKernelGGL(k_gemm_f32_grouped_linear, dim3(tiles + lin_blocks + pack_blocks), dim3(256), smem, st, g, job, tiles, lin_blocks, pk, 0);
+    hipLaunchKernelGGL(k_gemm_f32_grouped_linear, dim3(tiles + lin_blocks + pack_blocks), dim3(256), smem, st, g, job, tiles, lin_blocks, pk, pack_tab, 0);
     ORN_LAUNCH_CHECK("merge_group_linear");
     return 0;
 }
diff --git a/boosting-neural-video-representation-via-online-structural-reparameteration_amd/csrc/orn_merge_h16.hip b/boosting-neural-video-representation-via-online-structural-reparameteration_amd/csrc/orn_merge_h16.hip
--- a/boosting-neural-video-representation-via-online-structural-reparameteration_amd/csrc/orn_merge_h16.hip
+++ b/boosting-neural-video-representation-via-online-structural-reparameteration_amd/csrc/orn_merge_h16.hip
@@ -233,6 +233,12 @@
     return &H->pack;
 }
 
+void orn_merge_h16_grad_halfs(const void *host, int i, void **gh, void **gt, int *ldh, int *ldt)
+{
+    const MhPackLayer &l = ((const OrnMergeH16 *)host)->pack.l[i];
+    *gh = l.gh; *gt = l.gt; *ldh = r16(9 * l.C); *ldt = r16(l.O);
+}
+
 int orn_launch_merge_h16_pack_jobs(const void *host, int which, hipStream_t st)
 {
     const OrnMergeH16 *H = (const OrnMergeH16 *)host;
@@ -243,13 +249,15 @@
     return 0;
 }
 
-int orn_launch_merge_h16_bwd(const void *dev_tables, const void *host, hipStream_t st, OrnScaleState *sc)
+int orn_launch_merge_h16_bwd(const void *dev_tables, const void *host, hipStream_t st, OrnScaleState *sc, bool packed)
 {
     const OrnMergeH16 *H = (const OrnMergeH16 *)host;
     MhPackAll pack = H->pack;
     if (sc) pack.sc = sc;
-    hipLaunchKernelGGL(k_merge_pack, dim3(H->pack_blocks_grad), dim3(256), 0, st, pack, (int)MH_TAB_GRAD);
-    ORN_LAUNCH_CHECK("merge_pack");
+    if (!packed) {
+        hipLaunchKernelGGL(k_merge_pack, dim3(H->pack_blocks_grad), dim3(256), 0, st, pack, (int)MH_TAB_GRAD);
+        ORN_LAUNCH_CHECK("merge_pack");
+    }
     const MhGroup *g = (const MhGroup *)dev_tables;
     hipLaunchKernelGGL(k_mgemm_h16, dim3(H->tiles[0]), dim3(256), 0, st, g, H->tiles[0], pack.sc);
     ORN_LAUNCH_CHECK("mgemm_h16(dW3,dT)");
diff --git a/boosting-neural-video-representation-via-online-structural-reparameteration_amd/csrc/orn_wgrad_bf16.hip b/boosting-neural-video-representation-via-online-structural-reparameteration_amd/csrc/orn_wgrad_bf16.hip
--- a/boosting-neural-video-representation-via-online-structural-reparameteration_amd/csrc/orn_wgrad_bf16.hip
+++ b/boosting-neural-video-representation-via-online-structural-reparameteration_amd/csrc/orn_wgrad_bf16.hip
@@ -1,4 +1,5 @@
 #include "orn_h16.h"
+#include "orn_merge_pack.h"
 
 namespace HNS {
 
@@ -66,7 +67,8 @@
 
 __device__ __forceinline__ void wgrad_reduce_body(const float *__restrict__ slabs, const float *__restrict__ bias_slabs, int S, int O, int Cn,
                                                   int s2, int Cr, float gscale, float *__restrict__ dwf, float *__restrict__ dbf,
-                                                  OrnScaleState *sc = nullptr)
+                                                  OrnScaleState *sc = nullptr, mh16 *__restrict__ gh = nullptr, mh16 *__restrict__ gt = nullptr,
+                                                  int ldh = 0, int ldt = 0)
 {
     if (sc) gscale = sc->inv_gs;
     const size_t n = (size_t)9 * O * 96;
@@ -95,6 +97,13 @@
     const int o = nn * s2 + ij;
     dwf[((size_t)o * Cr + c) * 9 + tap] = acc * gscale;
     orn_flag_nonfinite(sc, acc * gscale);
+    if (gh) {
+        const mh16 hv = (mh16)((acc * gscale) * MH_GS);
+        const int e = c * 9 + tap;
+        gh[(size_t)o * ldh + e] = hv;
+        gt[(size_t)e * ldt + o] = hv;
+        if (!(fabsf((float)hv) <= 3.0e38f)) orn_flag_nonfinite(sc, __builtin_nanf(""));
+    }
 }
 
 __global__ void k_wgrad_bf16_reduce(const float *__restrict__ slabs, const float *__restrict__ bias_slabs, int S, int O, int Cn,
@@ -104,7 +113,7 @@
 }
 
 struct WgradReduceAll {
-    struct { const float *slabs, *bias_slabs; int S, O, Cn, s2, Cr; float gscale; float *dwf, *dbf; OrnScaleState *sc; } l[ORN_MAX_LAYERS];
+    struct { const float *slabs, *bias_slabs; int S, O, Cn, s2, Cr; float gscale; float *dwf, *dbf; OrnScaleState *sc; mh16 *gh, *gt; int ldh, ldt; } l[ORN_MAX_LAYERS];
     int n; OrnStemW0Job w0;
 };
 __global__ void k_wgrad_bf16_reduce_all(WgradReduceAll a)
@@ -118,7 +127,7 @@
     }
     const auto &l = a.l[blockIdx.y];
     if ((size_t)blockIdx.x * blockDim.x >= (size_t)9 * l.O * 96) return;
-    wgrad_reduce_body(l.slabs, l.bias_slabs, l.S, l.O, l.Cn, l.s2, l.Cr, l.gscale, l.dwf, l.dbf, l.sc);
+    wgrad_reduce_body(l.slabs, l.bias_slabs, l.S, l.O, l.Cn, l.s2, l.Cr, l.gscale, l.dwf, l.dbf, l.sc, l.gh, l.gt, l.ldh, l.ldt);
 }
 
 int orn_wgrad_bf16_split(int H, int W, int O, int smax = 0)
@@ -215,6 +224,7 @@
         a.l[i].slabs = L[i].slabs; a.l[i].bias_slabs = L[i].slabs + (size_t)S * 9 * L[i].O * 96;
         a.l[i].S = S; a.l[i].O = L[i].O; a.l[i].Cn = L[i].O / s2; a.l[i].s2 = s2; a.l[i].Cr = L[i].C; a.l[i].gscale = L[i].gscale;
         a.l[i].dwf = L[i].dwf; a.l[i].dbf = L[i].dbf; a.l[i].sc = L[i].sc;
+        a.l[i].gh = (mh16 *)L[i].gh; a.l[i].gt = (mh16 *)L[i].gt; a.l[i].ldh = L[i].ldh; a.l[i].ldt = L[i].ldt;
         const size_t w = (size_t)9 * L[i].O * 96;
         if (w > mx) mx = w;
     }
diff --git a/include/orn_debug.h b/include/orn_debug.h
--- a/include/orn_debug.h
+++ b/include/orn_debug.h
@@ -14,6 +14,7 @@
 ORN_API int orn_debug_conv_dgrad_f16(const void *dypad, const void *wd, int H, int W, int O, int C, const void *zprev,
                                      void *dyprev, int sp, float *dx_f32, int c_real, void *stream);
 ORN_API int orn_debug_merge_h16_bwd(int n, const int *co, const float *const *in, float *const *out, int *flag, void *stream);
+ORN_API int orn_debug_engine_grad_halfs(orn_engine *e, int layer, const void **gh, const void **gt, int *ldh, int *ldt);
 ORN_API size_t orn_debug_decode_out_ws_bytes(void);
 ORN_API int orn_debug_decode_out_f32(const float *img, int H, int W, const float *target, uint8_t *rgb8, float *img_out,
                                      float *stats, void *ws, size_t ws_bytes, void *stream);
```
